# hip-satomi/microbeSEG

Measured on AMD Instinct MI355X. Metric: training crops/sec (256px), higher is better.
Workload: dtype f32; 1 GPU; BASELINE configs[1]: DU-Net distance-map training step, filters [64, 1024], 256x256 crops, per-GPU batch 32, fp32, relu/bn, SmoothL1x2 + Adam(amsgrad); global_batch=32, parallelism=dp1, launch=eager

## Files before the change

### include/mseg_hip.h

```cpp
#ifndef MSEG_HIP_H
#define MSEG_HIP_H

#include <stddef.h>
#include <stdint.h>

#ifdef __cplusplus
extern "C" {
#endif

#define MSEG_OK 0
#define MSEG_EINVAL (-1)
#define MSEG_ELAUNCH (-2)
#define MSEG_EWORKSPACE (-3)

#define MSEG_ACT_NONE 0
#define MSEG_ACT_RELU 1
#define MSEG_ACT_LEAKY 2
#define MSEG_ACT_ELU 3
#define MSEG_ACT_MISH 4

#define MSEG_NORM_BN 0
#define MSEG_NORM_GN 1
#define MSEG_NORM_IN 2

#define MSEG_ST_F32 0
#define MSEG_ST_BF16 1
typedef struct MsegSrc {
  const float* ptr;
  const float* scale;
  const float* shift;
  int32_t C;
  int32_t act;
  int32_t ss;
  int32_t dtype;
} MsegSrc;

#define MSEG_MODE_CONV 0
#define MSEG_MODE_TCONV 1
#define MSEG_EPI_PLAIN 0
#define MSEG_EPI_SCATTER2X2 1
#define MSEG_MORDER_LINEAR 0
#define MSEG_MORDER_PARITY 1
#define MSEG_PREC_F32 0
#define MSEG_PREC_BF16 1

typedef struct MsegIgemm {
  MsegSrc src[2];
  const float* w;
  const float* bias;
  float* dst0;
  float* dst1;
  int32_t nsrc, Cin, Kpad, Npad;
  int32_t NB, Hi, Wi, Ho, Wo;
  int32_t KH, KW, stride, pad, mode, morder;
  int32_t Ngemm, epi, split, ld0, ld1, acc0, acc1, Cq;
  int32_t precision;
  int32_t dst_dtype;
  void* ws;
  size_t ws_bytes;
  float* stats;
  int32_t stats_act;
  int32_t reserved0;
} MsegIgemm;

int mseg_igemm(const MsegIgemm* p, void* stream);

typedef struct MsegKernelInfo {
  char name[120];
  int32_t precision;
  int32_t launches;
  uint32_t grid, block;
  size_t workspace;
  int32_t stats_rows;
  int32_t reserved0;
} MsegKernelInfo;
int mseg_igemm_query(const MsegIgemm* p, MsegKernelInfo* info);
const char* mseg_last_kernel(void);
int mseg_f32_to_bf16(const float* src, uint16_t* dst, size_t n, void* stream);
size_t mseg_igemm_workspace_bytes(const MsegIgemm* p);
int mseg_igemm_set_persistent(int on);
int mseg_igemm_set_wide_tiles(int on);
int mseg_igemm_set_p8(int mode);

typedef struct MsegWgrad {
  MsegSrc P;
  MsegSrc Q[2];
  float* ws;
  float* dst;
  int32_t nq, Nch, Nch_store;
  int32_t NB, Hp, Wp, Hq, Wq;
  int32_t KH, KW, stride, pad;
  int32_t splits;
  int32_t phase;
  int32_t precision;
  int32_t reserved;
} MsegWgrad;

size_t mseg_wgrad_workspace_bytes(const MsegWgrad* p);
int mseg_wgrad(const MsegWgrad* p, void* stream);
int mseg_wgrad_query(const MsegWgrad* p, MsegKernelInfo* info);

int mseg_first_conv_fwd(const float* x4, const float* w, const float* bias, int N, int H, int W, int Cin, int Cout,
                        void* z, int z_dtype, void* stream);
#define MSEG_PIX_U8 0
#define MSEG_PIX_U16 1
#define MSEG_PIX_I32 2
#define MSEG_PIX_F32 3
int mseg_frame_minmax(const void* raw, int dtype, size_t npix, uint32_t* minmax, void* stream);
int mseg_first_conv_fwd_raw(const void* raw, int dtype, int H0, int W0, int pad_top, int pad_left, const uint32_t* minmax,
                            const float* w, const float* bias, int Cout, void* z, int z_dtype, void* stream);
int mseg_frame_normalize(const void* raw, int dtype, int H0, int W0, int pad_top, int pad_left, const uint32_t* minmax,
                         float* out, void* stream);
int mseg_frames_minmax(const void* raw, int dtype, int N, size_t npix_per_frame, uint32_t* minmax, void* stream);
int mseg_frames_normalize(const void* raw, int dtype, int N, int H0, int W0, int pad_top, int pad_left,
                          const uint32_t* minmax, float* out, void* stream);
size_t mseg_first_wgrad_workspace_bytes(int N, int H, int W, int Cout);
int mseg_first_wgrad(const float* x4, const void* dz, int dz_dtype, int N, int H, int W, int Cout, float* dW, void* ws,
                     void* stream);

int mseg_pack_weight(const float* src, float* dst, int T, int R, int Rpad, int C, int Cpad, int st, int sr, int sc,
                     void* stream);

typedef struct MsegPackJob {
  const float* src;
  float* dst;
  uint16_t* dst16;
  int32_t T, R, Rpad, C, Cpad, st, sr, sc;
  uint32_t first_block;
  uint32_t reserved;
} MsegPackJob;
unsigned mseg_pack_job_blocks(int T, int Rpad, int Cpad);
int mseg_pack_weights_multi(const MsegPackJob* jobs_dev, int njobs, unsigned total_blocks, void* stream);

size_t mseg_norm_workspace_bytes(int N, int HW, int C);
int mseg_norm_set_tails(int on);
int mseg_norm_set_finish(int on);
int mseg_norm_stats(const void* z, int N, int HW, int C, int st, int act, int norm, const float* gamma,
                    const float* beta, float eps, float* scale, float* shift, float* mean, float* rstd,
                    float* running_mean, float* running_var, float momentum, void* act_out, void* ws, void* stream);
int mseg_norm_stats_from_conv(const float* part, int rows, int C, long long count, const float* gamma, const float* beta,
                              float eps, float* scale, float* shift, float* mean, float* rstd, float* running_mean,
                              float* running_var, float momentum, void* ws, void* stream);
int mseg_activation(const void* z, int N, int HW, int C, int st, int act, void* act_out, void* stream);
int mseg_bn_eval_coeffs(const float* gamma, const float* beta, const float* running_mean,
                        const float* running_var, float eps, int C, float* scale, float* shift, void* stream);
int mseg_norm_bwd(const void* gy, const void* z, int N, int HW, int C, int st, int act, int norm, const float* gamma,
                  const float* mean, const float* rstd, void* dz, float* dgamma, float* dbeta, float* dbias,
                  const void* act_in , void* ws, void* stream);

int mseg_maxpool2x2_fwd(const MsegSrc* src, int N, int H, int W, float* out, void* stream);
int mseg_maxpool2x2_bwd(const MsegSrc* src, int N, int H, int W, const float* gout, float* gin, int accumulate,
                        void* stream);

int mseg_head_fwd(const MsegSrc* src, int N, int HW, const float* w, const float* b, int Co, float* out_nchw,
                  void* stream);
size_t mseg_head_bwd_workspace_bytes(int N, int HW, int C, int Co);
int mseg_head_bwd(const MsegSrc* src, int N, int HW, const float* w, int Co, const float* gout_nchw, void* gy,
                  int gy_dtype , float* dW, float* db, void* ws,
                  void* stream);

int mseg_softmax3_hwc(const float* logits_chw, int Hp, int Wp, int pad_y, int pad_x, float* probs_hwc, void* stream);

size_t mseg_loss_workspace_bytes(size_t n);
int mseg_regression_loss(const float* pred, const float* target, size_t n, int kind, float* loss_out,
                         void* ws, void* stream);
int mseg_regression_loss_bwd(const float* pred, const float* target, size_t n, int kind, const float* gscale_dev,
                             float* grad, void* stream);
int mseg_ce_dice_fwd(const float* logits, const int64_t* labels, int N, int HW, int with_dice, double* sums6,
                     double* ce_sum, void* ws, void* stream);
int mseg_ce_dice_bwd(const float* logits, const int64_t* labels, int N, int HW, int with_dice, const double* sums6,
                     double total_px, double dice_weight, const float* gscale_dev, float* grad, void* stream);

int mseg_polygons_find(const uint16_t* labels, int H, int W, int32_t* cand_px, int32_t* cand_id, int32_t* cand_len,
                       int capacity, int32_t* n_cand_dev, void* stream);
int mseg_polygons_trace(const uint16_t* labels, int H, int W, const int32_t* start_px, const int64_t* offsets, int n_poly,
                        int32_t* points_yx, void* stream);

int mseg_adam_amsgrad_step(float* p, const float* g, float* m, float* v, float* vmax, size_t n, double lr,
                           double beta1, double beta2, double eps, int step, void* stream);
int mseg_adam_amsgrad_step_dev(float* p, const float* g, float* m, float* v, float* vmax, size_t n, double* state,
                               double beta1, double beta2, double eps, void* stream);
int mseg_ranger_step(float* p, const float* g, float* m, float* v, float* slow, size_t n, int rows, double beta1,
                     double beta2, double eps, double step_lr, int rectified, int do_gc, int lookahead, double alpha,
                     void* stream);
typedef struct MsegRangerJob {
  float* p;
  const float* g;
  float* m;
  float* v;
  float* slow;
  uint64_t n;
  int32_t rows;
  float step_lr;
  uint32_t flags;
  uint32_t reserved;
} MsegRangerJob;
int mseg_ranger_step_multi(const MsegRangerJob* jobs, int njobs, double beta1, double beta2, double eps, double alpha,
                           void* stream);

size_t mseg_postproc_workspace_bytes(int H, int W);
int mseg_postproc_tuning(int heap_rows, int tile_small_px, int tile_large_px);
int mseg_postproc_set_const_stream(int on);
int mseg_distance_postprocess(const float* border, const float* cell, int H, int W, float th_cell, float th_seed,
                              int col_major_ids, uint16_t* labels, int32_t* n_instances_dev, int32_t* status_dev,
                              void* ws, size_t ws_bytes, void* stream);
int mseg_boundary_postprocess(const float* probs_hwc, int H, int W, uint16_t* labels, int32_t* n_instances_dev,
                              int32_t* status_dev, void* ws, size_t ws_bytes, void* stream);
int mseg_boundary_postprocess_pre(const float* probs_hwc, int H, int W, void* ws, size_t ws_bytes, void* stream);
int mseg_boundary_flood_batch(void* const* ws_list, int B, int H, int W, void* stream);
int mseg_boundary_postprocess_post(int H, int W, uint16_t* labels, int32_t* n_instances_dev, int32_t* status_dev, void* ws,
                                   size_t ws_bytes, void* stream);

int mseg_distance_postprocess_sweep(const float* border, const float* cell, int H, int W, const float* th_cell,
                                    const float* th_seed, int nth, int col_major_ids, uint16_t* labels,
                                    int32_t* n_instances_dev, int32_t* status_dev, void* ws, size_t ws_bytes,
                                    void* stream);

size_t mseg_postproc_batch_workspace_bytes(int N, int H, int W);
int mseg_distance_postprocess_batch(const float* border, const float* cell, int N, int H, int W, long long row_stride,
                                    long long frame_stride, float th_cell, float th_seed, int col_major_ids,
                                    uint16_t* labels, int32_t* n_instances_dev, int32_t* status_dev, void* ws,
                                    size_t ws_bytes, void* stream);

int mseg_aug_u16_to_f32(const uint16_t* in, float* out, size_t n, void* stream);
int mseg_aug_flip(const float* in, float* out, int N, int H, int W, const int32_t* codes_dev, void* stream);
int mseg_aug_affine(const float* in, float* out, int N, int H, int W, const float* mats_dev, const int32_t* apply_dev,
                    int nearest, void* stream);
int mseg_aug_blur(const float* in, float* tmp, float* out, int N, int H, int W, const float* sigmas_dev, void* stream);
int mseg_aug_stats(const float* in, int N, int H, int W, float* stats_dev, uint32_t* hist_dev, void* stream);
int mseg_aug_contrast_params(const float* stats_dev, const uint32_t* hist_dev, const float* choice_dev, int N, int HW,
                             float* par_dev, void* stream);
// ... 63 lines not shown
```

### microbeseg_amd/_lib.py

```python
import ctypes as C
import os
import pathlib

_HERE = pathlib.Path(__file__).resolve().parent
LIB_PATH = _HERE / "libmseg_hip.so"

ACT = {"none": 0, "relu": 1, "leakyrelu": 2, "elu": 3, "mish": 4}
NORM = {"bn": 0, "gn": 1, "in": 2}
MODE_CONV, MODE_TCONV = 0, 1
EPI_PLAIN, EPI_SCATTER2X2 = 0, 1
MORDER_LINEAR, MORDER_PARITY = 0, 1
ST_F32, ST_BF16 = 0, 1
PIX_U8, PIX_U16, PIX_I32, PIX_F32 = 0, 1, 2, 3


class MsegLibraryError(RuntimeError):
    pass


class MsegSrc(C.Structure):
    _fields_ = [("ptr", C.c_void_p), ("scale", C.c_void_p), ("shift", C.c_void_p),
                ("C", C.c_int32), ("act", C.c_int32), ("ss", C.c_int32), ("dtype", C.c_int32)]


class MsegIgemm(C.Structure):
    _fields_ = [("src", MsegSrc * 2), ("w", C.c_void_p), ("bias", C.c_void_p), ("dst0", C.c_void_p),
                ("dst1", C.c_void_p),
                ("nsrc", C.c_int32), ("Cin", C.c_int32), ("Kpad", C.c_int32), ("Npad", C.c_int32),
                ("NB", C.c_int32), ("Hi", C.c_int32), ("Wi", C.c_int32), ("Ho", C.c_int32), ("Wo", C.c_int32),
                ("KH", C.c_int32), ("KW", C.c_int32), ("stride", C.c_int32), ("pad", C.c_int32),
                ("mode", C.c_int32), ("morder", C.c_int32),
                ("Ngemm", C.c_int32), ("epi", C.c_int32), ("split", C.c_int32), ("ld0", C.c_int32),
                ("ld1", C.c_int32), ("acc0", C.c_int32), ("acc1", C.c_int32), ("Cq", C.c_int32),
                ("precision", C.c_int32), ("dst_dtype", C.c_int32), ("ws", C.c_void_p), ("ws_bytes", C.c_size_t),
                ("stats", C.c_void_p), ("stats_act", C.c_int32), ("reserved0", C.c_int32)]


class MsegWgrad(C.Structure):
    _fields_ = [("P", MsegSrc), ("Q", MsegSrc * 2), ("ws", C.c_void_p), ("dst", C.c_void_p),
                ("nq", C.c_int32), ("Nch", C.c_int32), ("Nch_store", C.c_int32),
                ("NB", C.c_int32), ("Hp", C.c_int32), ("Wp", C.c_int32), ("Hq", C.c_int32), ("Wq", C.c_int32),
                ("KH", C.c_int32), ("KW", C.c_int32), ("stride", C.c_int32), ("pad", C.c_int32),
                ("splits", C.c_int32), ("phase", C.c_int32), ("precision", C.c_int32), ("reserved", C.c_int32)]


class MsegKernelInfo(C.Structure):
    _fields_ = [("name", C.c_char * 120), ("precision", C.c_int32), ("launches", C.c_int32), ("grid", C.c_uint32),
                ("block", C.c_uint32), ("workspace", C.c_size_t), ("stats_rows", C.c_int32), ("reserved0", C.c_int32)]


class MsegPackJob(C.Structure):
    _fields_ = [("src", C.c_void_p), ("dst", C.c_void_p), ("dst16", C.c_void_p),
                ("T", C.c_int32), ("R", C.c_int32), ("Rpad", C.c_int32), ("C", C.c_int32), ("Cpad", C.c_int32),
                ("st", C.c_int32), ("sr", C.c_int32), ("sc", C.c_int32),
                ("first_block", C.c_uint32), ("reserved", C.c_uint32)]


class MsegRangerJob(C.Structure):
    _fields_ = [("p", C.c_void_p), ("g", C.c_void_p), ("m", C.c_void_p), ("v", C.c_void_p), ("slow", C.c_void_p),
                ("n", C.c_uint64), ("rows", C.c_int32), ("step_lr", C.c_float), ("flags", C.c_uint32),
                ("reserved", C.c_uint32)]


_P = C.c_void_p
_I = C.c_int
_F = C.c_float
_D = C.c_double
_SZ = C.c_size_t

SIGNATURES = {
    "mseg_igemm": (_I, [C.POINTER(MsegIgemm), _P]),
    "mseg_igemm_workspace_bytes": (_SZ, [C.POINTER(MsegIgemm)]),
    "mseg_igemm_query": (_I, [C.POINTER(MsegIgemm), C.POINTER(MsegKernelInfo)]),
    "mseg_last_kernel": (C.c_char_p, []),
    "mseg_igemm_set_persistent": (_I, [_I]),
    "mseg_igemm_set_wide_tiles": (_I, [_I]),
    "mseg_igemm_set_p8": (_I, [_I]),
    "mseg_f32_to_bf16": (_I, [_P, _P, _SZ, _P]),
    "mseg_first_conv_fwd": (_I, [_P, _P, _P, _I, _I, _I, _I, _I, _P, _I, _P]),
    "mseg_frame_minmax": (_I, [_P, _I, _SZ, _P, _P]),
    "mseg_first_conv_fwd_raw": (_I, [_P, _I, _I, _I, _I, _I, _P, _P, _P, _I, _P, _I, _P]),
    "mseg_frame_normalize": (_I, [_P, _I, _I, _I, _I, _I, _P, _P, _P]),
    "mseg_frames_minmax": (_I, [_P, _I, _I, _SZ, _P, _P]),
    "mseg_frames_normalize": (_I, [_P, _I, _I, _I, _I, _I, _I, _P, _P, _P]),
    "mseg_first_wgrad_workspace_bytes": (_SZ, [_I, _I, _I, _I]),
    "mseg_first_wgrad": (_I, [_P, _P, _I, _I, _I, _I, _I, _P, _P, _P]),
    "mseg_wgrad_workspace_bytes": (_SZ, [C.POINTER(MsegWgrad)]),
    "mseg_wgrad": (_I, [C.POINTER(MsegWgrad), _P]),
    "mseg_wgrad_query": (_I, [C.POINTER(MsegWgrad), C.POINTER(MsegKernelInfo)]),
    "mseg_pack_weight": (_I, [_P, _P, _I, _I, _I, _I, _I, _I, _I, _I, _P]),
    "mseg_pack_job_blocks": (C.c_uint, [_I, _I, _I]),
    "mseg_pack_weights_multi": (_I, [_P, _I, C.c_uint, _P]),
    "mseg_norm_workspace_bytes": (_SZ, [_I, _I, _I]),
    "mseg_norm_set_tails": (_I, [_I]),
    "mseg_norm_set_finish": (_I, [_I]),
    "mseg_norm_stats_from_conv": (_I, [_P, _I, _I, C.c_longlong, _P, _P, _F, _P, _P, _P, _P, _P, _P, _F, _P, _P]),
    "mseg_norm_stats": (_I, [_P, _I, _I, _I, _I, _I, _I, _P, _P, _F, _P, _P, _P, _P, _P, _P, _F, _P, _P, _P]),
    "mseg_activation": (_I, [_P, _I, _I, _I, _I, _I, _P, _P]),
    "mseg_bn_eval_coeffs": (_I, [_P, _P, _P, _P, _F, _I, _P, _P, _P]),
    "mseg_norm_bwd": (_I, [_P, _P, _I, _I, _I, _I, _I, _I, _P, _P, _P, _P, _P, _P, _P, _P, _P, _P]),
    "mseg_maxpool2x2_fwd": (_I, [C.POINTER(MsegSrc), _I, _I, _I, _P, _P]),
    "mseg_maxpool2x2_bwd": (_I, [C.POINTER(MsegSrc), _I, _I, _I, _P, _P, _I, _P]),
    "mseg_head_fwd": (_I, [C.POINTER(MsegSrc), _I, _I, _P, _P, _I, _P, _P]),
    "mseg_head_bwd_workspace_bytes": (_SZ, [_I, _I, _I, _I]),
    "mseg_head_bwd": (_I, [C.POINTER(MsegSrc), _I, _I, _P, _I, _P, _P, _I, _P, _P, _P, _P]),
    "mseg_softmax3_hwc": (_I, [_P, _I, _I, _I, _I, _P, _P]),
    "mseg_loss_workspace_bytes": (_SZ, [_SZ]),
    "mseg_regression_loss": (_I, [_P, _P, _SZ, _I, _P, _P, _P]),
    "mseg_regression_loss_bwd": (_I, [_P, _P, _SZ, _I, _P, _P, _P]),
    "mseg_ce_dice_fwd": (_I, [_P, _P, _I, _I, _I, _P, _P, _P, _P]),
    "mseg_ce_dice_bwd": (_I, [_P, _P, _I, _I, _I, _P, C.c_double, C.c_double, _P, _P, _P]),
    "mseg_adam_amsgrad_step": (_I, [_P, _P, _P, _P, _P, _SZ, _D, _D, _D, _D, _I, _P]),
    "mseg_adam_amsgrad_step_dev": (_I, [_P, _P, _P, _P, _P, _SZ, _P, _D, _D, _D, _P]),
    "mseg_ranger_step": (_I, [_P, _P, _P, _P, _P, _SZ, _I, _D, _D, _D, _D, _I, _I, _I, _D, _P]),
    "mseg_ranger_step_multi": (_I, [_P, _I, _D, _D, _D, _D, _P]),
    "mseg_postproc_workspace_bytes": (_SZ, [_I, _I]),
    "mseg_postproc_tuning": (_I, [_I, _I, _I]),
    "mseg_postproc_set_const_stream": (_I, [_I]),
    "mseg_distance_postprocess": (_I, [_P, _P, _I, _I, _F, _F, _I, _P, _P, _P, _P, _SZ, _P]),
    "mseg_boundary_postprocess": (_I, [_P, _I, _I, _P, _P, _P, _P, _SZ, _P]),
    "mseg_boundary_postprocess_pre": (_I, [_P, _I, _I, _P, _SZ, _P]),
    "mseg_boundary_flood_batch": (_I, [C.POINTER(C.c_void_p), _I, _I, _I, _P]),
    "mseg_boundary_postprocess_post": (_I, [_I, _I, _P, _P, _P, _P, _SZ, _P]),
    "mseg_distance_postprocess_sweep": (_I, [_P, _P, _I, _I, C.POINTER(C.c_float), C.POINTER(C.c_float), _I, _I, _P, _P,
                                             _P, _P, _SZ, _P]),
    "mseg_postproc_batch_workspace_bytes": (_SZ, [_I, _I, _I]),
    "mseg_distance_postprocess_batch": (_I, [_P, _P, _I, _I, _I, C.c_longlong, C.c_longlong, _F, _F, _I, _P, _P, _P, _P,
                                             _SZ, _P]),
    "mseg_aug_u16_to_f32": (_I, [_P, _P, _SZ, _P]),
    "mseg_aug_flip": (_I, [_P, _P, _I, _I, _I, _P, _P]),
    "mseg_aug_affine": (_I, [_P, _P, _I, _I, _I, _P, _P, _I, _P]),
    "mseg_aug_blur": (_I, [_P, _P, _P, _I, _I, _I, _P, _P]),
    "mseg_aug_stats": (_I, [_P, _I, _I, _I, _P, _P, _P]),
    "mseg_aug_contrast_params": (_I, [_P, _P, _P, _I, _I, _P, _P]),
    "mseg_aug_contrast": (_I, [_P, _P, _I, _I, _I, _P, _P]),
    "mseg_aug_clahe_workspace_bytes": (_SZ, [_I]),
    "mseg_aug_clahe": (_I, [_P, _P, _I, _I, _I, _P, _P, _P]),
    "mseg_aug_noise_normalize": (_I, [_P, _P, _I, _I, _I, _P, _P, C.c_uint32, _F, _F, _P]),
    "mseg_clahe_workspace_bytes": (_SZ, [_I, _I, _I]),
    "mseg_clahe_u16": (_I, [_P, _I, _I, _I, _I, _P, _P, _I, _P, _SZ, _P]),
    "mseg_label_boundary": (_I, [_P, _I, _I, _I, _I, _P, _P]),
    "mseg_label_distance_workspace_bytes": (_SZ, [_I, _I, _I]),
    "mseg_label_distance": (_I, [_P, _I, _I, _I, _I, _P, _P, _P, _SZ, _P]),
    "mseg_label_bottom_hat": (_I, [_P, _I, _I, _I, _P, _P, _P, _SZ, _P]),
    "mseg_label_cell_distance": (_I, [_P, _I, _I, _I, _I, _F, _P, _P, _SZ, _P]),
    "mseg_label_j4": (_I, [_P, _I, _I, _I, _I, _I, _P, _P, _P]),
    "mseg_label_major_axis_workspace_bytes": (_SZ, [_I]),
    "mseg_label_max_major_axis": (_I, [_P, _I, _I, _I, _P, _P, _SZ, _P]),
    "mseg_eval_workspace_bytes": (_SZ, [_I, _I]),
    "mseg_eval_relabel": (_I, [_P, _I, _I, _I, _P, _P, _P, _SZ, _P]),
    "mseg_eval_pair_counts": (_I, [_P, _P, _I, _I, _I, _I, _P, _P, _P, _P]),
    "mseg_polygons_find": (_I, [_P, _I, _I, _P, _P, _P, _I, _P, _P]),
    "mseg_polygons_trace": (_I, [_P, _I, _I, _P, _P, _I, _P, _P]),
    "mseg_roi_fill_workspace_bytes": (_SZ, [_I]),
    "mseg_roi_fill": (_I, [_P, _P, _P, _I, _I, _I, _I, _P, _P, _SZ, _P]),
    "mseg_roi_outline": (_I, [_P, _P, _P, _I, C.c_int64, _I, _I, _I, _P, _P]),
    "mseg_stack_relabel_workspace_bytes": (_SZ, [_I, _I, _I]),
    "mseg_stack_relabel": (_I, [_P, _I, _I, _I, _I, _P, _P, _P, _SZ, _P]),
    "mseg_region_stats_workspace_bytes": (_SZ, [C.c_int64]),
    "mseg_region_stats": (_I, [_P, _I, _I, _I, _P, C.c_int64, _P, _P, _P, _P, _P, _SZ, _P]),
    "mseg_overlay_workspace_bytes": (_SZ, []),
    "mseg_overlay_rgb": (_I, [_P, _I, _I, _I, _I, _I, _P, _P, _P, _SZ, _P]),
    "mseg_frame_stats": (_I, [_P, _I, _SZ, _P, _P]),
    "mseg_crops_extract": (_I, [_P, _I, _I, _I, _I, _P, _I, _I, _I, _I, _P, _P, _P, _P, _P]),
    "mseg_crop_census_workspace_bytes": (_SZ, []),
    "mseg_crop_census": (_I, [_P, _I, _I, _I, _I, _I, _I, _I, _I, _P, _P, _P, _SZ, _P]),
    "mseg_crops_overlay": (_I, [_P, _P, _P, _I, _I, _P]),
    "mseg_version": (_I, []),
    "mseg_strerror": (C.c_char_p, [_I]),
    "mseg_last_hip_error": (_I, []),
}

_lib = None


def load():
    global _lib
    if _lib is not None:
        return _lib
    import torch
    path = os.environ.get("MSEG_HIP_LIB", str(LIB_PATH))
    if not os.path.exists(path):
        raise MsegLibraryError(
# ... 24 lines not shown
```

### microbeseg_amd/csrc/api_misc.hip

```cpp
#include "common.h"
#include <string.h>

static thread_local int g_last_hip_error = 0;

extern "C" void mseg_set_hip_error(int e) { g_last_hip_error = e; }
extern "C" int mseg_last_hip_error(void) { return g_last_hip_error; }
extern "C" int mseg_version(void) { return 100; }
extern "C" const char* mseg_strerror(int code) {
  switch (code) {
    case MSEG_OK: return "ok";
    case MSEG_EINVAL: return "invalid argument or unsupported shape";
    case MSEG_ELAUNCH: return "HIP launch/runtime error (see mseg_last_hip_error)";
    case MSEG_EWORKSPACE: return "workspace too small";
    default: return "unknown error";
  }
}

static thread_local int g_dry = 0;
static thread_local MsegKernelInfo g_call;
static thread_local char g_last_kernel[sizeof(g_call.name)] = "";

extern "C" int mseg_dispatch_dry(void) { return g_dry; }
extern "C" void mseg_dispatch_begin(int dry) {
  g_dry = dry;
  memset(&g_call, 0, sizeof(g_call));
}
extern "C" void mseg_dispatch_end(MsegKernelInfo* info) {
  if (!g_dry && g_call.name[0]) memcpy(g_last_kernel, g_call.name, sizeof(g_last_kernel));
  if (info) *info = g_call;
  g_dry = 0;
}
extern "C" void mseg_dispatch_note(int precision, size_t workspace) {
  g_call.precision = precision;
  g_call.workspace = workspace;
}
extern "C" void mseg_dispatch_note_stats(int rows) { g_call.stats_rows = rows; }
extern "C" void mseg_note_launch(const char* kernel, unsigned grid, unsigned block, int aux) {
  g_call.launches += 1;
  if (aux || g_call.name[0]) return;
  size_t n = strlen(kernel);
  if (n >= 2 && kernel[0] == '(' && kernel[n - 1] == ')') { ++kernel; n -= 2; }
  if (n >= sizeof(g_call.name)) n = sizeof(g_call.name) - 1;
  memcpy(g_call.name, kernel, n);
  g_call.name[n] = 0;
  g_call.grid = grid;
  g_call.block = block;
}
extern "C" const char* mseg_last_kernel(void) { return g_last_kernel; }
```

### microbeseg_amd/csrc/common.h

```cpp
#pragma once
#include <hip/hip_runtime.h>
#include <stdint.h>
#include "../../include/mseg_hip.h"

extern "C" void mseg_set_hip_error(int e);
extern "C" int mseg_dispatch_dry(void);

#define MSEG_LAUNCH_CHECK()                           \
  do {                                                \
    if (mseg_dispatch_dry()) break;                   \
    hipError_t e__ = hipGetLastError();               \
    if (e__ != hipSuccess) {                          \
      mseg_set_hip_error((int)e__);                   \
      return MSEG_ELAUNCH;                            \
    }                                                 \
  } while (0)

extern "C" void mseg_note_launch(const char* kernel, unsigned grid, unsigned block, int aux);
extern "C" void mseg_dispatch_begin(int dry);
extern "C" void mseg_dispatch_end(MsegKernelInfo* info);
extern "C" void mseg_dispatch_note(int precision, size_t workspace);
extern "C" void mseg_dispatch_note_stats(int rows);
#define MSEG_KL(K, grid_, block_, shmem_, st_, ...)                                              \
  do {                                                                                           \
    mseg_note_launch(#K, (unsigned)(grid_).x, (unsigned)(block_).x, 0);                          \
    if (!mseg_dispatch_dry()) hipLaunchKernelGGL(K, grid_, block_, shmem_, st_, ##__VA_ARGS__);    \
  } while (0)
#define MSEG_KL_AUX(K, grid_, block_, shmem_, st_, ...)                                          \
  do {                                                                                           \
    mseg_note_launch(#K, (unsigned)(grid_).x, (unsigned)(block_).x, 1);                          \
    if (!mseg_dispatch_dry()) hipLaunchKernelGGL(K, grid_, block_, shmem_, st_, ##__VA_ARGS__);    \
  } while (0)

typedef float f32x16 __attribute__((ext_vector_type(16)));
typedef float f32x4 __attribute__((ext_vector_type(4)));

__device__ __forceinline__ float mseg_softplus(float x) {
  return x > 20.f ? x : log1pf(expf(x));
}

template <bool FAST>
__device__ __forceinline__ float mish_fwd(float x) {
  if (x > 20.f) return x;
  const float w = FAST ? __expf(x) : expf(x);
  const float n = w * (w + 2.f);
  return FAST ? x * n * __frcp_rn(n + 2.f) : x * (n / (n + 2.f));
}
template <bool FAST>
__device__ __forceinline__ float mish_bwd(float x) {
  if (x > 20.f) return 1.f;
  const float w = FAST ? __expf(x) : expf(x);
  const float n = w * (w + 2.f);
  const float r = FAST ? __frcp_rn(n + 2.f) : 1.f / (n + 2.f);
  return n * r + 4.f * x * w * (w + 1.f) * r * r;
}

template <int ACT>
__device__ __forceinline__ float act_fwd_t(float x) {
  if (ACT == MSEG_ACT_RELU) return x > 0.f ? x : 0.f;
  if (ACT == MSEG_ACT_LEAKY) return x > 0.f ? x : 0.01f * x;
  if (ACT == MSEG_ACT_ELU) return x > 0.f ? x : expm1f(x);
  if (ACT == MSEG_ACT_MISH) return mish_fwd<false>(x);
  return x;
}

__device__ __forceinline__ float act_fwd(float x, int act) {
  switch (act) {
    case MSEG_ACT_RELU: return act_fwd_t<MSEG_ACT_RELU>(x);
    case MSEG_ACT_LEAKY: return act_fwd_t<MSEG_ACT_LEAKY>(x);
    case MSEG_ACT_ELU: return act_fwd_t<MSEG_ACT_ELU>(x);
    case MSEG_ACT_MISH: return act_fwd_t<MSEG_ACT_MISH>(x);
    default: return x;
  }
}

__device__ __forceinline__ float act_bwd(float z, int act) {
  switch (act) {
    case MSEG_ACT_RELU: return z > 0.f ? 1.f : 0.f;
    case MSEG_ACT_LEAKY: return z > 0.f ? 1.f : 0.01f;
    case MSEG_ACT_ELU: return z > 0.f ? 1.f : expf(z);
    case MSEG_ACT_MISH: return mish_bwd<false>(z);
    default: return 1.f;
  }
}

__device__ __forceinline__ float act_fwd_fast(float x, int act) {
  if (act == MSEG_ACT_MISH) return mish_fwd<true>(x);
  if (act == MSEG_ACT_ELU) return x > 0.f ? x : __expf(x) - 1.f;
  return act_fwd(x, act);
}
__device__ __forceinline__ float act_bwd_fast(float z, int act) {
  if (act == MSEG_ACT_MISH) return mish_bwd<true>(z);
  if (act == MSEG_ACT_ELU) return z > 0.f ? 1.f : __expf(z);
  return act_bwd(z, act);
}

template <bool FAST>
__device__ __forceinline__ void act_pair(float z, int act, float& a, float& d) {
  if (act == MSEG_ACT_MISH) {
    if (z > 20.f) { a = z; d = 1.f; return; }
    const float w = FAST ? __expf(z) : expf(z);
    const float n = w * (w + 2.f);
    if (FAST) {
      const float r = __frcp_rn(n + 2.f);
      a = z * n * r;
      d = n * r + 4.f * z * w * (w + 1.f) * r * r;
    } else {
      const float r = 1.f / (n + 2.f);
      a = z * (n / (n + 2.f));
      d = n * r + 4.f * z * w * (w + 1.f) * r * r;
    }
    return;
  }
  a = FAST ? act_fwd_fast(z, act) : act_fwd(z, act);
  d = FAST ? act_bwd_fast(z, act) : act_bwd(z, act);
}

__device__ __forceinline__ float4 act_fwd4(float4 v, int act) {
  if (act == MSEG_ACT_NONE) return v;
  if (act == MSEG_ACT_RELU) {
    v.x = fmaxf(v.x, 0.f); v.y = fmaxf(v.y, 0.f); v.z = fmaxf(v.z, 0.f); v.w = fmaxf(v.w, 0.f);
    return v;
  }
  v.x = act_fwd(v.x, act); v.y = act_fwd(v.y, act); v.z = act_fwd(v.z, act); v.w = act_fwd(v.w, act);
  return v;
}

__device__ __forceinline__ float4 src_load4(const MsegSrc& s, size_t e);

__device__ __forceinline__ float4 src_transform4(float4 v, const MsegSrc& s, int n, int c) {
  v = act_fwd4(v, s.act);
  if (s.scale) {
    const float4 sc = *reinterpret_cast<const float4*>(s.scale + (size_t)n * s.ss + c);
    const float4 sh = *reinterpret_cast<const float4*>(s.shift + (size_t)n * s.ss + c);
    v.x = v.x * sc.x + sh.x; v.y = v.y * sc.y + sh.y; v.z = v.z * sc.z + sh.z; v.w = v.w * sc.w + sh.w;
  }
  return v;
}

typedef __bf16 mseg_bf16x2 __attribute__((ext_vector_type(2)));

__device__ __forceinline__ float bf16_lo(unsigned v) { return __uint_as_float(v << 16); }
__device__ __forceinline__ float bf16_hi(unsigned v) { return __uint_as_float(v & 0xffff0000u); }
__device__ __forceinline__ unsigned pack_bf16x2(float a, float b) {
  mseg_bf16x2 v;
  v[0] = (__bf16)a; v[1] = (__bf16)b;
  return __builtin_bit_cast(unsigned, v);
}
__device__ __forceinline__ float4 bf16x4_to_f32(uint2 v) {
  return make_float4(bf16_lo(v.x), bf16_hi(v.x), bf16_lo(v.y), bf16_hi(v.y));
}
__device__ __forceinline__ uint2 f32x4_to_bf16(float4 v) { return make_uint2(pack_bf16x2(v.x, v.y), pack_bf16x2(v.z, v.w)); }

template <bool S16>
__device__ __forceinline__ float4 ld_f4(const void* base, size_t e) {
  if (S16) return bf16x4_to_f32(*reinterpret_cast<const uint2*>(reinterpret_cast<const uint16_t*>(base) + e));
  return *reinterpret_cast<const float4*>(reinterpret_cast<const float*>(base) + e);
}
template <bool S16>
__device__ __forceinline__ void st_f4(void* base, size_t e, float4 v) {
  if (S16) *reinterpret_cast<uint2*>(reinterpret_cast<uint16_t*>(base) + e) = f32x4_to_bf16(v);
  else *reinterpret_cast<float4*>(reinterpret_cast<float*>(base) + e) = v;
}
__device__ __forceinline__ float4 ld_f4_rt(const void* base, size_t e, int bf16) {
  return bf16 ? ld_f4<true>(base, e) : ld_f4<false>(base, e);
}
// ... 31 lines not shown
```

### microbeseg_amd/csrc/igemm.hip

```cpp
#include "common.h"
#include "igemm_common.h"
#include "bf16_affine.h"

int igemm_p8_try(const MsegIgemm& p, int tr, int m_fastest, int cus, hipStream_t st);

__device__ float g_ident_scale[MSEG_MAX_CH];
__device__ float g_ident_shift[MSEG_MAX_CH];
__global__ void init_ident_kernel() {
  for (int i = blockIdx.x * blockDim.x + threadIdx.x; i < MSEG_MAX_CH; i += gridDim.x * blockDim.x) {
    g_ident_scale[i] = 1.f;
    g_ident_shift[i] = 0.f;
  }
}


template <int BM, int BN, bool PER_SAMPLE, bool GENERIC_ACT>
__global__ __launch_bounds__(256) void igemm_kernel(const MsegIgemm p) {
  using Cfg = IgemmCfg<BM, BN>;
  constexpr int STAGE = (BM + BN) * LDS_STRIDE;
  __shared__ __attribute__((aligned(16))) float lds[2 * STAGE + 4];
  unsigned* tapmask_s = reinterpret_cast<unsigned*>(lds + 2 * STAGE);

  const int tid = threadIdx.x;
  const int lane = tid & 63;
// ... 357 lines not shown
      const int cls = m0 / (M >> 2);
      py = cls >> 1; px = cls & 1;
    }
    for (int tt = 0; tt < T; ++tt) {
      const int ky_ = tt / p.KW, kx_ = tt - ky_ * p.KW;
      const bool live = (((py - geom.dir * (ky_ - geom.pad)) | (px - geom.dir * (kx_ - geom.pad))) & geom.sh) == 0;
      if (live) {
        const unsigned long long e = (unsigned long long)(tt | (ky_ << 4) | (kx_ << 6));
        if (nlive < 8) taplist |= e << (8 * nlive); else taplist_hi |= e << (8 * (nlive - 8));
        ++nlive;
      }
    }
  }
  auto tap_at = [&](int j) -> unsigned { return (unsigned)((j < 8 ? taplist >> (8 * j) : taplist_hi >> (8 * (j - 8))) & 0xffull); };
  int chunk = 0, j = 0;
  const int nsteps = nchunks * nlive;
  unsigned e0 = tap_at(0);
  issue(0, (int)(e0 & 15u), (int)((e0 >> 4) & 3u), (int)(e0 >> 6));
  commit(lds, lds + BM * LDS_STRIDE);
  __syncthreads();
  int cur = 0;
  const int li = lane & 31, lh = lane >> 5;
  for (int step = 0; step < nsteps; ++step) {
    if (step + 1 < nsteps) {
      j += 1;
      if (j >= nlive) { j = 0; ++chunk; }
    }
    e0 = tap_at(j);
    issue(chunk, (int)(e0 & 15u), (int)((e0 >> 4) & 3u), (int)(e0 >> 6));

    const float* As = lds + cur * STAGE;
    const float* Bs = As + BM * LDS_STRIDE;
#pragma unroll
    for (int kk = 0; kk < KC / 8; ++kk) {
      float4 af[Cfg::MB], bf[Cfg::NB];
#pragma unroll
      for (int a = 0; a < Cfg::MB; ++a)
        af[a] = *reinterpret_cast<const float4*>(As + (wm * Cfg::TM + a * 32 + li) * LDS_STRIDE + kk * 8 + lh * 4);
#pragma unroll
      for (int b = 0; b < Cfg::NB; ++b)
        bf[b] = *reinterpret_cast<const float4*>(Bs + (wn * Cfg::TN + b * 32 + li) * LDS_STRIDE + kk * 8 + lh * 4);
#pragma unroll
      for (int a = 0; a < Cfg::MB; ++a)
#pragma unroll
        for (int b = 0; b < Cfg::NB; ++b) {
          acc[a][b] = __builtin_amdgcn_mfma_f32_32x32x2f32(af[a].x, bf[b].x, acc[a][b], 0, 0, 0);
          acc[a][b] = __builtin_amdgcn_mfma_f32_32x32x2f32(af[a].y, bf[b].y, acc[a][b], 0, 0, 0);
          acc[a][b] = __builtin_amdgcn_mfma_f32_32x32x2f32(af[a].z, bf[b].z, acc[a][b], 0, 0, 0);
          acc[a][b] = __builtin_amdgcn_mfma_f32_32x32x2f32(af[a].w, bf[b].w, acc[a][b], 0, 0, 0);
        }
    }
    if (SB) {
      __syncthreads();
      commit(lds, lds + BM * LDS_STRIDE);
      __syncthreads();
    } else {
      float* An = lds + (cur ^ 1) * STAGE;
      commit(An, An + BM * LDS_STRIDE);
      __syncthreads();
      cur ^= 1;
    }
  }
  igemm_epilogue<IgemmCfg<BM, BN>>(acc, m0, n0, wm, wn, lane, M);
}

template <int BN>
struct HaloCfg {
  static constexpr int WN = (BN >= 128) ? 4 : 2;
  static constexpr int WM = 8 / WN;
  static constexpr int TM = 128 / WM, TN = BN / WN;
  static constexpr int MB = TM / 32, NB = TN / 32;
  static constexpr int BROWS = BN / 64;
};

template <int BN, int TR>
__global__ __launch_bounds__(512, 2) void igemm_halo_kernel(const MsegIgemm p, int tw_log2, int ksplit,
                                                            int chunks_per_split) {
  constexpr int BM = 128;
  using Cfg = HaloCfg<BN>;
  constexpr int HMAX = 264;
  constexpr int HL = (HMAX * 8 + 511) / 512;
  constexpr int ASTAGE = HMAX * LDS_STRIDE;
  constexpr int BSTAGE = BN * LDS_STRIDE;
  __shared__ __attribute__((aligned(16))) float lds[ASTAGE + 2 * BSTAGE];
  float* const Abuf = lds;
  float* const Bbuf = lds + ASTAGE;

  const int tid = threadIdx.x, lane = tid & 63, wave = tid >> 6;
  const int wm = wave / Cfg::WN, wn = wave % Cfg::WN;
  const int li = lane & 31, lh = lane >> 5;
  const int srow = tid >> 3, scol = tid & 7;
  const int TW = 1 << tw_log2, TH = BM >> tw_log2, HW2 = TW + 2;
  const int HROWS = (TH + 2) * HW2;
  const int H = p.Hi, W = p.Wi;
  const int M = p.NB * H * W;
  const int tiles_x = W >> tw_log2, tiles_y = (H + TH - 1) / TH;
  const int ntiles_n = (p.Ngemm + BN - 1) / BN;
  const int lid_all = (int)xcd_logical_id(blockIdx.x, gridDim.x);
  const int ntiles_all = (int)gridDim.x / ksplit;
  const int kz = lid_all / ntiles_all;
  const int lid = lid_all - kz * ntiles_all;
  const int tile_m = lid / ntiles_n, tile_n = lid - tile_m * ntiles_n;
  const int img = tile_m / (tiles_x * tiles_y);
  const int trem = tile_m - img * (tiles_x * tiles_y);
  const int ty = trem / tiles_x, tx = trem - ty * tiles_x;
  const int oy0 = ty * TH, ox0 = tx * TW, n0 = tile_n * BN;
  const int band0 = oy0 > 0 ? oy0 - 1 : 0;
  const int band_rows = (oy0 + TH + 1 < H ? oy0 + TH + 1 : H) - band0;
  const bool conv = p.mode == MSEG_MODE_CONV;

  int hpix[HL];
  unsigned hvalid = 0u;
#pragma unroll
  for (int j = 0; j < HL; ++j) {
    const int hrow = srow + 64 * j;
    const int hy = hrow / HW2, hx = hrow - hy * HW2;
    const int iy = oy0 - 1 + hy, ix = ox0 - 1 + hx;
    const bool ok = (hrow < HROWS) & (iy >= 0) & (iy < H) & (ix >= 0) & (ix < W);
    hpix[j] = (iy - band0) * W + ix;
    hvalid |= (unsigned)ok << j;
  }
  int abase[Cfg::MB];
#pragma unroll
  for (int a = 0; a < Cfg::MB; ++a) {
    const int i = wm * Cfg::TM + a * 32 + li;
    abase[a] = ((i >> tw_log2) * HW2 + (i & (TW - 1))) * LDS_STRIDE + lh * 4;
  }

  f32x16 acc[Cfg::MB][Cfg::NB];
#pragma unroll
  for (int a = 0; a < Cfg::MB; ++a)
#pragma unroll
    for (int b = 0; b < Cfg::NB; ++b)
#pragma unroll
      for (int r = 0; r < 16; ++r) acc[a][b][r] = 0.f;

  const int nchunks = (p.Cin + KC - 1) / KC;
  const int C0 = p.src[0].C;
  const unsigned OOB = 0x80000000u;
  const int C1 = p.nsrc > 1 ? p.src[1].C : p.src[0].C;
  const float* const base0 = p.src[0].ptr + ((size_t)img * H + band0) * W * p.src[0].C;
  const float* const base1 = (p.nsrc > 1 ? p.src[1].ptr : p.src[0].ptr) + ((size_t)img * H + band0) * W * C1;
  const __amdgpu_buffer_rsrc_t rs0 = __builtin_amdgcn_make_buffer_rsrc(const_cast<float*>(base0), 0,
                                                                        band_rows * W * p.src[0].C * 4, 0x00020000);
  const __amdgpu_buffer_rsrc_t rs1 = __builtin_amdgcn_make_buffer_rsrc(const_cast<float*>(base1), 0,
                                                                        band_rows * W * C1 * 4, 0x00020000);
  const __amdgpu_buffer_rsrc_t rsw = __builtin_amdgcn_make_buffer_rsrc(const_cast<float*>(p.w), 0,
                                                                        9 * p.Npad * p.Kpad * 4, 0x00020000);
  unsigned wvoff[Cfg::BROWS];
#pragma unroll
  for (int i = 0; i < Cfg::BROWS; ++i) wvoff[i] = ((unsigned)(n0 + srow + 64 * i) * (unsigned)p.Kpad + scol * 4u) * 4u;

  float4 rh[HL], rb[Cfg::BROWS], rsc, rsh;
  unsigned hlive = 0u;
  int ract = 0;
  bool cur_s1 = false;

  auto issue_halo = [&](int chunk) {
    const int c = chunk * KC + scol * 4;
    cur_s1 = (p.nsrc > 1) && (chunk * KC >= C0);
    const MsegSrc& s = cur_s1 ? p.src[1] : p.src[0];
    const unsigned sC4 = (unsigned)s.C * 4u;
    const unsigned soff = (unsigned)(chunk * KC - (cur_s1 ? C0 : 0)) * 4u + scol * 16u;
    hlive = (c < p.Cin) ? hvalid : 0u;
#pragma unroll
    for (int j = 0; j < HL; ++j) {
      const bool ok = (hlive >> j) & 1u;
      const unsigned vo = ok ? (unsigned)hpix[j] * sC4 + soff : OOB;
      const f32x4 v = cur_s1 ? __builtin_bit_cast(f32x4, __builtin_amdgcn_raw_buffer_load_b128(rs1, vo, 0, 0))
                             : __builtin_bit_cast(f32x4, __builtin_amdgcn_raw_buffer_load_b128(rs0, vo, 0, 0));
      rh[j] = make_float4(v[0], v[1], v[2], v[3]);
    }
    if (TR != 0) {
      ract = s.act;
      const bool has_aff = s.scale != nullptr;
      const float* scp = has_aff ? s.scale : g_ident_scale;
      const float* shp = has_aff ? s.shift : g_ident_shift;
      const unsigned cl = (c < p.Cin) ? (unsigned)(cur_s1 ? c - C0 : c) : 0u;
      const size_t o = (size_t)img * (has_aff ? (unsigned)s.ss : 0u) + cl;
      rsc = *reinterpret_cast<const float4*>(scp + o);
      rsh = *reinterpret_cast<const float4*>(shp + o);
    }
  };

  auto commit_halo = [&](float* As) {
    const float lo = (ract == MSEG_ACT_RELU) ? 0.f : -3.402823466e38f;
#pragma unroll
    for (int j = 0; j < HL; ++j) {
      const int hrow = srow + 64 * j;
      if (hrow < HMAX) {
        float4 v = rh[j];
        if (TR != 0) {
          if (TR == 2) v = act_fwd4(v, ract);
          else { v.x = clamp_lo(v.x, lo); v.y = clamp_lo(v.y, lo); v.z = clamp_lo(v.z, lo); v.w = clamp_lo(v.w, lo); }
          const float m = ((hlive >> j) & 1u) ? 1.f : 0.f;
          v.x = (v.x * rsc.x + rsh.x) * m; v.y = (v.y * rsc.y + rsh.y) * m;
          v.z = (v.z * rsc.z + rsh.z) * m; v.w = (v.w * rsc.w + rsh.w) * m;
        }
        *reinterpret_cast<float4*>(As + hrow * LDS_STRIDE + scol * 4) = v;
      }
    }
  };

  auto issue_b = [&](int chunk, int t) {
    const unsigned wso = ((unsigned)t * (unsigned)p.Npad * (unsigned)p.Kpad + (unsigned)chunk * KC) * 4u;
#pragma unroll
    for (int i = 0; i < Cfg::BROWS; ++i) {
      const f32x4 v = __builtin_bit_cast(f32x4, __builtin_amdgcn_raw_buffer_load_b128(rsw, wvoff[i], wso, 0));
      rb[i] = make_float4(v[0], v[1], v[2], v[3]);
    }
  };
  auto commit_b = [&](float* Bs) {
#pragma unroll
    for (int i = 0; i < Cfg::BROWS; ++i)
      *reinterpret_cast<float4*>(Bs + (srow + 64 * i) * LDS_STRIDE + scol * 4) = rb[i];
  };

  const int c_begin = kz * chunks_per_split;
  const int c_end = (c_begin + chunks_per_split < nchunks) ? c_begin + chunks_per_split : nchunks;
  issue_halo(c_begin);
  issue_b(c_begin, 0);
  commit_halo(Abuf);
  commit_b(Bbuf);
  __syncthreads();

  int bsel = 0;
  for (int chunk = c_begin; chunk < c_end; ++chunk) {
    const float* As = Abuf;
    const bool more_chunks = chunk + 1 < c_end;
    for (int t = 0; t < 9; ++t) {
      if (t == 0 && more_chunks) issue_halo(chunk + 1);
      const bool last = (t == 8) && !more_chunks;
      issue_b(t == 8 ? (more_chunks ? chunk + 1 : chunk) : chunk, last ? 8 : (t == 8 ? 0 : t + 1));

      const int ky = t / 3, kx = t - 3 * ky;
      const int toff = ((conv ? ky : 2 - ky) * HW2 + (conv ? kx : 2 - kx)) * LDS_STRIDE;
      const float* Bs = Bbuf + bsel * BSTAGE;
#pragma unroll
      for (int kk = 0; kk < KC / 8; ++kk) {
        float4 af[Cfg::MB], bf[Cfg::NB];
#pragma unroll
        for (int a = 0; a < Cfg::MB; ++a)
          af[a] = *reinterpret_cast<const float4*>(As + abase[a] + toff + kk * 8);
#pragma unroll
        for (int b = 0; b < Cfg::NB; ++b)
          bf[b] = *reinterpret_cast<const float4*>(Bs + (wn * Cfg::TN + b * 32 + li) * LDS_STRIDE + kk * 8 + lh * 4);
#pragma unroll
        for (int a = 0; a < Cfg::MB; ++a)
#pragma unroll
          for (int b = 0; b < Cfg::NB; ++b) {
            acc[a][b] = __builtin_amdgcn_mfma_f32_32x32x2f32(af[a].x, bf[b].x, acc[a][b], 0, 0, 0);
            acc[a][b] = __builtin_amdgcn_mfma_f32_32x32x2f32(af[a].y, bf[b].y, acc[a][b], 0, 0, 0);
            acc[a][b] = __builtin_amdgcn_mfma_f32_32x32x2f32(af[a].z, bf[b].z, acc[a][b], 0, 0, 0);
            acc[a][b] = __builtin_amdgcn_mfma_f32_32x32x2f32(af[a].w, bf[b].w, acc[a][b], 0, 0, 0);
          }
      }
      commit_b(Bbuf + (bsel ^ 1) * BSTAGE);
      if (t == 8 && more_chunks) {
        __syncthreads();
        commit_halo(Abuf);
      }
      __syncthreads();
      bsel ^= 1;
    }
  }
  igemm_epilogue<Cfg>(acc, 0, n0, wm, wn, lane, M * ksplit, tw_log2, img + kz * p.NB, oy0, ox0);
}

typedef __bf16 bf16x8 __attribute__((ext_vector_type(8)));
typedef __bf16 bf16x4 __attribute__((ext_vector_type(4)));
#define HB_STRIDE 40

template <int BN, int BM>
struct HaloCfgM {
  static constexpr int WN = (BN >= 128) ? 4 : 2;
  static constexpr int WM = 8 / WN;
  static constexpr int TM = BM / WM, TN = BN / WN;
  static constexpr int MB = TM / 32, NB = TN / 32;
  static constexpr int BROWS = BN / 64;
};

template <int BN, int TR, bool S16, int BM>
__device__ __forceinline__ void igemm_halo_bf16_body(const MsegIgemm& p, int tw_log2, int ksplit, int chunks_per_split,
                                                     int m_fastest) {
  using Cfg = HaloCfgM<BN, BM>;
  constexpr int HMAX = BM == 128 ? 204 : 612;
  constexpr int SQ = S16 ? 4 : 8;
  constexpr int SROWS = 512 / SQ;
  constexpr int HL = (HMAX + SROWS - 1) / SROWS;
  constexpr int ASTAGE = HMAX * HB_STRIDE;
  constexpr int BSTAGE = 3 * BN * HB_STRIDE;
  __shared__ __attribute__((aligned(16))) __bf16 lds[ASTAGE + 2 * BSTAGE];
  __bf16* const Abuf = lds;
  __bf16* const Bbuf = lds + ASTAGE;

  const int tid = threadIdx.x, lane = tid & 63, wave = tid >> 6;
  const int wm = wave / Cfg::WN, wn = wave % Cfg::WN;
  const int li = lane & 31, lh = lane >> 5;
  const int srow = tid / SQ, scol = tid % SQ;
  const int brow = tid >> 2, bcol = tid & 3;
  const int TW = 1 << tw_log2, TH = BM >> tw_log2, HW2 = TW + 2;
  const int HROWS = (TH + 2) * HW2;
  const int H = p.Hi, W = p.Wi;
  const int M = p.NB * H * W;
  const int tiles_x = W >> tw_log2, tiles_y = (H + TH - 1) / TH;
  const int ntiles_n = (p.Ngemm + BN - 1) / BN;
  const int lid_all = (int)xcd_logical_id(blockIdx.x, gridDim.x);
  const int ntiles_all = (int)gridDim.x / ksplit;
  const int kz = lid_all / ntiles_all;
  const int lid = lid_all - kz * ntiles_all;
  const int ntiles_m = ntiles_all / ntiles_n;
  const int tile_m = m_fastest ? lid % ntiles_m : lid / ntiles_n;
  const int tile_n = m_fastest ? lid / ntiles_m : lid - tile_m * ntiles_n;
// ... 1750 lines not shown
  if (ks <= 1 || (p.Ngemm & 3)) return 0;
  return (size_t)ks * p.NB * p.Hi * p.Wi * p.Ngemm * sizeof(float);
}

static int igemm_dispatch(const MsegIgemm* pp, void* stream) {
  if (!pp) return MSEG_EINVAL;
  const MsegIgemm& p = *pp;
  if (p.nsrc < 1 || p.nsrc > 2) return MSEG_EINVAL;
  int csum = 0;
  for (int i = 0; i < p.nsrc; ++i) {
    if (check_src(p.src[i])) return MSEG_EINVAL;
    csum += p.src[i].C;
  }
  if (csum != p.Cin) return MSEG_EINVAL;
  if (!p.w || !p.dst0 || p.Kpad < p.Cin || (p.Kpad % KC) || p.Npad < p.Ngemm || (p.Npad % 128)) return MSEG_EINVAL;
  if (p.Cin > MSEG_MAX_CH) return MSEG_EINVAL;
  if (p.NB <= 0 || p.Hi <= 0 || p.Wi <= 0 || p.Ho <= 0 || p.Wo <= 0) return MSEG_EINVAL;
  if (p.KH <= 0 || p.KW <= 0 || p.KH * p.KW > 16) return MSEG_EINVAL;
  if (p.stride != 1 && p.stride != 2) return MSEG_EINVAL;
  if (p.mode != MSEG_MODE_CONV && p.mode != MSEG_MODE_TCONV) return MSEG_EINVAL;
  if (p.morder == MSEG_MORDER_PARITY && ((p.Ho | p.Wo) & 1)) return MSEG_EINVAL;
  if (p.Ngemm <= 0) return MSEG_EINVAL;
  if (p.precision != MSEG_PREC_F32 && p.precision != MSEG_PREC_BF16) return MSEG_EINVAL;
  if (p.dst_dtype != MSEG_ST_F32 && p.dst_dtype != MSEG_ST_BF16) return MSEG_EINVAL;
  const bool s16 = p.src[0].dtype == MSEG_ST_BF16;
  if (p.nsrc > 1 && p.src[1].dtype != p.src[0].dtype) return MSEG_EINVAL;
  if ((s16 || p.dst_dtype == MSEG_ST_BF16) && p.precision != MSEG_PREC_BF16) return MSEG_EINVAL;
  if (p.dst_dtype == MSEG_ST_BF16) {
    if ((p.Ngemm | p.ld0 | p.ld1 | p.Cq) & 1) return MSEG_EINVAL;
    if (p.split < p.Ngemm && (p.split & 1)) return MSEG_EINVAL;
    if (((uintptr_t)p.dst0 | (uintptr_t)p.dst1) & 3) return MSEG_EINVAL;
  }
  if (p.epi == MSEG_EPI_SCATTER2X2) {
    if (p.Cq <= 0 || p.Ngemm != 4 * p.Cq || p.morder != MSEG_MORDER_LINEAR) return MSEG_EINVAL;
  } else if (p.epi == MSEG_EPI_PLAIN) {
    if (p.split < p.Ngemm && !p.dst1) return MSEG_EINVAL;
  } else {
    return MSEG_EINVAL;
  }
  const long long M = (long long)p.NB * p.Ho * p.Wo;
  if (M <= 0 || M > 0x7fffffffLL) return MSEG_EINVAL;
  hipStream_t st = (hipStream_t)stream;
  mseg_dispatch_note(p.precision, 0);
  static bool ident_ready[64] = {false};
  int devid = 0;
  const bool dry = mseg_dispatch_dry() != 0;
  if (!dry) {
    if (hipGetDevice(&devid) != hipSuccess || devid < 0 || devid >= 64) return MSEG_ELAUNCH;
    if (!ident_ready[devid]) {
      MSEG_KL_AUX(init_ident_kernel, dim3(8), dim3(256), 0, st);
      MSEG_LAUNCH_CHECK();
      ident_ready[devid] = true;
    }
  }
  bool per_sample = false, generic = false;
  for (int i = 0; i < p.nsrc; ++i) {
    if (p.src[i].scale && p.src[i].ss != 0) per_sample = true;
    if (p.src[i].act != MSEG_ACT_NONE && p.src[i].act != MSEG_ACT_RELU) generic = true;
  }
  const bool wide = p.Ngemm > 64;
  const int BMv = 128, BNv = wide ? 128 : 64;
  const long long tiles = ((M + BMv - 1) / BMv) * ((p.Ngemm + BNv - 1) / BNv);
  if (tiles > 0x7fffffffLL) return MSEG_EINVAL;
  const dim3 grid((unsigned)tiles), block(256);
  bool fast = (p.mode == MSEG_MODE_CONV) || (p.stride == 1) ||
              (p.morder == MSEG_MORDER_PARITY && (M % (4 * BMv)) == 0);
  bool plain = true, band_fits = true;
  for (int i = 0; i < p.nsrc; ++i) {
    if (((128LL / p.Wo + 3) * p.stride + p.KH) * p.Wi * p.src[i].C * 4 >= 0x7ffffff0LL) fast = false;
    if (34LL * p.Wi * p.src[i].C * 4 >= 0x80000000LL) band_fits = false;
    if (p.src[i].act != MSEG_ACT_NONE || p.src[i].scale) plain = false;
  }
  bool common = true;
  if ((long long)p.KH * p.KW * p.Npad * p.Kpad * 4 >= 0x80000000LL) common = false;
  if (p.KH > 4 || p.KW > 4) common = false;
  if (p.nsrc > 1 && (p.src[0].C % KC)) common = false;
  fast = fast && common;
  int tw_log2 = 6;
  long long htiles = 0;
  if (common && band_fits && halo_geometry(p, BNv, &tw_log2, &htiles) && htiles <= 0x7fffffffLL) {
    const int tr = plain ? 0 : (generic ? 2 : 1);
    int cps = 0;
    int ks = halo_ksplit(htiles, (p.Cin + KC - 1) / KC, &cps);
    const size_t need = (size_t)ks * (size_t)M * (size_t)p.Ngemm * sizeof(float);
    if (ks > 1 && (!p.ws || p.ws_bytes < need || (p.Ngemm & 3) || (p.split & 3) || htiles * ks > 0x7fffffffLL)) {
      ks = 1;
      cps = (p.Cin + KC - 1) / KC;
    }
    MsegIgemm q = p;
    if (ks > 1) {
      q.dst0 = (float*)p.ws; q.dst1 = nullptr; q.ld0 = p.Ngemm; q.ld1 = 0; q.split = p.Ngemm; q.acc0 = 0; q.acc1 = 0;
      q.bias = nullptr;
      q.dst_dtype = MSEG_ST_F32;
    }
    mseg_dispatch_note(p.precision, ks > 1 ? need : 0);
    const dim3 hgrid((unsigned)(htiles * ks));
#define MSEG_HALO(BN_, TR_) MSEG_KL((igemm_halo_kernel<BN_, TR_>), hgrid, dim3(512), 0, st, q, tw_log2, ks, cps)
    const int m_fastest = ((long long)9 * p.Kpad * p.Ngemm * 2 > (2ll << 20)) && (p.Ngemm > BNv) ? 1 : 0;
#define MSEG_HALO16(BN_, TR_)                                                                                          \
  do {                                                                                                                 \
    if (s16) MSEG_KL((igemm_halo_bf16_kernel<BN_, TR_, true>), hgrid, dim3(512), 0, st, q, tw_log2, ks, cps, m_fastest); \
    else MSEG_KL((igemm_halo_bf16_kernel<BN_, TR_, false>), hgrid, dim3(512), 0, st, q, tw_log2, ks, cps, m_fastest);    \
  } while (0)
#define MSEG_HALO16W4(TR_)                                                                                             \
  do {                                                                                                                 \
    if (s16) MSEG_KL((igemm_halo_bf16w4_kernel<TR_, true>), hgrid, dim3(256), 0, st, q, tw_log2, ks, cps, m_fastest);    \
    else MSEG_KL((igemm_halo_bf16w4_kernel<TR_, false>), hgrid, dim3(256), 0, st, q, tw_log2, ks, cps, m_fastest);       \
  } while (0)
    int p8rc = 0;
    if (p.precision == MSEG_PREC_BF16 && s16 && !wide && g_c64p_on && p.nsrc == 1 && p.Cin == 64 && p.Kpad == 64 &&
        ks == 1 && tw_log2 <= 5 && p.split >= p.Ngemm && htiles >= 4 * (long long)c64p_workgroups()) {
      const int wgs = c64p_workgroups();
      const dim3 pgrid((unsigned)wgs);
#define MSEG_C64P(TR_)                                                                                                        \
  do {                                                                                                                         \
    if (q.dst_dtype == MSEG_ST_BF16) MSEG_KL((igemm_c64p_bf16_kernel<TR_, true>), pgrid, dim3(512), 0, st, q, tw_log2, (int)htiles); \
    else MSEG_KL((igemm_c64p_bf16_kernel<TR_, false>), pgrid, dim3(512), 0, st, q, tw_log2, (int)htiles);               \
  } while (0)
      if (tr == 0) MSEG_C64P(0); else if (tr == 1) MSEG_C64P(1); else MSEG_C64P(2);
#undef MSEG_C64P
    } else if (p.precision == MSEG_PREC_BF16 && !wide && g_c64p_on && p.Cin >= 128 && ks == 1 && tw_log2 >= 4 &&
               halo512_tiles(p, tw_log2) >= 2 * (long long)c64p_workgroups()) {
      const dim3 mgrid((unsigned)halo512_tiles(p, tw_log2));
#define MSEG_HALO512(TR_)                                                                                                      \
  do {                                                                                                                         \
    if (s16) MSEG_KL((igemm_halo_bf16m512_kernel<TR_, true>), mgrid, dim3(512), 0, st, q, tw_log2, 1, cps, 0);      \
    else MSEG_KL((igemm_halo_bf16m512_kernel<TR_, false>), mgrid, dim3(512), 0, st, q, tw_log2, 1, cps, 0);         \
  } while (0)
      if (tr == 0) MSEG_HALO512(0); else if (tr == 1) MSEG_HALO512(1); else MSEG_HALO512(2);
#undef MSEG_HALO512
    } else if (p.precision == MSEG_PREC_BF16 && wide && s16 && ks == 1 &&
               (p8rc = igemm_p8_try(q, tr, m_fastest, c64p_workgroups(), st)) != 0) {
      if (p8rc < 0) return p8rc;
    } else if (p.precision == MSEG_PREC_BF16 && wide && s16 && g_w4m_on && ks == 1 && tw_log2 >= 3 &&
               halo_big_tiles(p, tw_log2, 256) * ((p.Ngemm + 127) / 128) >= 2 * (long long)c64p_workgroups()) {
      const dim3 mgrid((unsigned)(halo_big_tiles(p, tw_log2, 256) * ((p.Ngemm + 127) / 128)));
#define MSEG_HALOW4M(TR_) \
  MSEG_KL((igemm_halo_bf16w4m_kernel<TR_, true>), mgrid, dim3(256), 0, st, q, tw_log2, 1, cps, m_fastest)
      if (tr == 0) MSEG_HALOW4M(0); else if (tr == 1) MSEG_HALOW4M(1); else MSEG_HALOW4M(2);
#undef MSEG_HALOW4M
    } else if (p.precision == MSEG_PREC_BF16) {
      if (wide) { if (tr == 0) MSEG_HALO16W4(0); else if (tr == 1) MSEG_HALO16W4(1); else MSEG_HALO16W4(2); }
      else      { if (tr == 0) MSEG_HALO16(64, 0); else if (tr == 1) MSEG_HALO16(64, 1); else MSEG_HALO16(64, 2); }
    } else if (wide) { if (tr == 0) MSEG_HALO(128, 0); else if (tr == 1) MSEG_HALO(128, 1); else MSEG_HALO(128, 2); }
    else      { if (tr == 0) MSEG_HALO(64, 0); else if (tr == 1) MSEG_HALO(64, 1); else MSEG_HALO(64, 2); }
#undef MSEG_HALO
#undef MSEG_HALO16
#undef MSEG_HALO16W4
    MSEG_LAUNCH_CHECK();
    if (ks > 1) {
      const size_t total = (size_t)M * (size_t)(p.Ngemm >> 2);
      size_t blocks = (total + 255) / 256;
      if (blocks > 16384) blocks = 16384;
      MSEG_KL_AUX(igemm_splitk_reduce_kernel, dim3((unsigned)blocks), dim3(256), 0, st, (const float*)p.ws, ks,
                         (size_t)M, p.Ngemm, p.bias, p.dst0, p.ld0, p.acc0, p.dst1, p.ld1, p.acc1,
                         p.split < p.Ngemm ? p.split : p.Ngemm, p.dst_dtype == MSEG_ST_BF16 ? 1 : 0);
      MSEG_LAUNCH_CHECK();
    }
    return MSEG_OK;
  }
  if (p.precision == MSEG_PREC_BF16 && s16 && g_c64p_on && p.epi == MSEG_EPI_SCATTER2X2 && p.KH == 1 && p.KW == 1 &&
      p.stride == 1 && p.pad == 0 && p.mode == MSEG_MODE_CONV && p.nsrc == 1 && p.Cin == 128 && p.Kpad == 128 &&
      p.Cq == 64 && p.Ngemm == 256 && !p.acc0 && (p.Wi % 32) == 0 && (((long long)p.Hi * p.Wi) % 128) == 0 &&
      M / 128 >= 4 * (long long)c64p_workgroups()) {
    const int tr = plain ? 0 : (generic ? 2 : 1);
    const dim3 pgrid((unsigned)c64p_workgroups());
    const int nt = (int)(M / 128);
#define MSEG_CTP(TR_)                                                                                                \
  do {                                                                                                               \
    if (p.dst_dtype == MSEG_ST_BF16) MSEG_KL((igemm_ctp_bf16_kernel<TR_, true>), pgrid, dim3(512), 0, st, p, nt); \
    else MSEG_KL((igemm_ctp_bf16_kernel<TR_, false>), pgrid, dim3(512), 0, st, p, nt);                     \
  } while (0)
    if (tr == 0) MSEG_CTP(0); else if (tr == 1) MSEG_CTP(1); else MSEG_CTP(2);
#undef MSEG_CTP
    MSEG_LAUNCH_CHECK();
    return MSEG_OK;
  }
  if (p.precision == MSEG_PREC_BF16 && s16 && g_c64p_on && p.epi == MSEG_EPI_SCATTER2X2 && p.KH == 1 && p.KW == 1 &&
      p.stride == 1 && p.pad == 0 && p.mode == MSEG_MODE_CONV && p.nsrc == 1 && p.Cin == 256 && p.Kpad == 256 &&
      p.Cq == 128 && p.Ngemm == 512 && !p.acc0 && p.Wi >= 32 && (((long long)p.Hi * p.Wi) % 64) == 0 &&
      (c64p_workgroups() & 3) == 0 && M / 64 >= 4 * (long long)(c64p_workgroups() / 4)) {
    const int tr = plain ? 0 : (generic ? 2 : 1);
    const dim3 pgrid((unsigned)c64p_workgroups());
    const int nt = (int)(M / 64);
#define MSEG_CTP2(TR_)                                                                                               \
  do {                                                                                                               \
    if (p.dst_dtype == MSEG_ST_BF16) MSEG_KL((igemm_ctp2_bf16_kernel<TR_, true>), pgrid, dim3(512), 0, st, p, nt); \
    else MSEG_KL((igemm_ctp2_bf16_kernel<TR_, false>), pgrid, dim3(512), 0, st, p, nt);                    \
  } while (0)
    if (tr == 0) MSEG_CTP2(0); else if (tr == 1) MSEG_CTP2(1); else MSEG_CTP2(2);
#undef MSEG_CTP2
    MSEG_LAUNCH_CHECK();
    return MSEG_OK;
  }
  if (p.precision == MSEG_PREC_BF16 && s16 && g_c64p_on && plain && p.epi == MSEG_EPI_PLAIN && p.KH == 2 && p.KW == 2 &&
      p.stride == 2 && p.pad == 0 && p.mode == MSEG_MODE_CONV && p.morder == MSEG_MORDER_LINEAR && p.nsrc == 1 &&
      p.Cin == 64 && p.Kpad == 64 && p.Ngemm == 128 && p.split >= p.Ngemm && !p.acc0 && !p.bias && (p.Wo % 32) == 0 &&
      p.Hi == 2 * p.Ho && p.Wi == 2 * p.Wo && (M % 64) == 0 && M / 64 >= 4 * (long long)c64p_workgroups()) {
    const dim3 pgrid((unsigned)c64p_workgroups());
    if (p.dst_dtype == MSEG_ST_BF16) MSEG_KL((igemm_ctd_bf16_kernel<true>), pgrid, dim3(512), 0, st, p, (int)(M / 64));
    else MSEG_KL((igemm_ctd_bf16_kernel<false>), pgrid, dim3(512), 0, st, p, (int)(M / 64));
    MSEG_LAUNCH_CHECK();
    return MSEG_OK;
  }
  if (p.precision == MSEG_PREC_BF16) {
    if (!fast) return MSEG_EINVAL;
    const int tr = plain ? 0 : (generic ? 2 : 1);
#define MSEG_FAST16_LAUNCH(BM_, BN_, TR_, PS_)                                                          \
  do {                                                                                                  \
    if (s16) MSEG_KL((igemm_fast_bf16_kernel<BM_, BN_, TR_, PS_, true>), grid, block, 0, st, p);   \
    else MSEG_KL((igemm_fast_bf16_kernel<BM_, BN_, TR_, PS_, false>), grid, block, 0, st, p);      \
  } while (0)
#define MSEG_FAST16_TILE(BM_, BN_)                                                        \
  do {                                                                                    \
    if (tr == 0) MSEG_FAST16_LAUNCH(BM_, BN_, 0, false);                                  \
    else if (tr == 1) { if (per_sample) MSEG_FAST16_LAUNCH(BM_, BN_, 1, true); else MSEG_FAST16_LAUNCH(BM_, BN_, 1, false); } \
    else { if (per_sample) MSEG_FAST16_LAUNCH(BM_, BN_, 2, true); else MSEG_FAST16_LAUNCH(BM_, BN_, 2, false); }              \
  } while (0)
    if (wide) MSEG_FAST16_TILE(128, 128); else MSEG_FAST16_TILE(128, 64);
#undef MSEG_FAST16_TILE
#undef MSEG_FAST16_LAUNCH
    MSEG_LAUNCH_CHECK();
    return MSEG_OK;
  }
  if (fast) {
    const int tr = plain ? 0 : (generic ? 2 : 1);
    const int live_taps = (p.mode == MSEG_MODE_TCONV && p.stride == 2) ? ((p.KH + 1) / 2) * ((p.KW + 1) / 2) : p.KH * p.KW;
    const bool short_k = ((p.Cin + KC - 1) / KC) * live_taps <= 8;
#define MSEG_FAST_LAUNCH(BM_, BN_, TR_, PS_)                                                              \
  do {                                                                                                    \
    if (short_k) MSEG_KL((igemm_fast_kernel<BM_, BN_, TR_, PS_, true>), grid, block, 0, st, p); \
    else MSEG_KL((igemm_fast_kernel<BM_, BN_, TR_, PS_, false>), grid, block, 0, st, p);        \
  } while (0)
#define MSEG_FAST_TILE(BM_, BN_)                                                          \
  do {                                                                                    \
    if (tr == 0) MSEG_FAST_LAUNCH(BM_, BN_, 0, false);                                    \
    else if (tr == 1) { if (per_sample) MSEG_FAST_LAUNCH(BM_, BN_, 1, true); else MSEG_FAST_LAUNCH(BM_, BN_, 1, false); } \
    else { if (per_sample) MSEG_FAST_LAUNCH(BM_, BN_, 2, true); else MSEG_FAST_LAUNCH(BM_, BN_, 2, false); }              \
  } while (0)
    if (wide) MSEG_FAST_TILE(128, 128); else MSEG_FAST_TILE(128, 64);
#undef MSEG_FAST_TILE
#undef MSEG_FAST_LAUNCH
    MSEG_LAUNCH_CHECK();
// ... 122 lines not shown
```

### microbeseg_amd/csrc/norm.hip

```cpp
#include "common.h"
#include <stdlib.h>

struct NormGeom {
  int N, HW, C, chunks, rows_per_chunk;
  int cw, slices;
};

#define NORM_CTR_BYTES 65536
#define NORM_CTR_MAX (NORM_CTR_BYTES / 4)

static NormGeom norm_geom(int N, int HW, int C, int vec = 4) {
  NormGeom g;
  g.N = N; g.HW = HW; g.C = C;
  const int C4 = C / vec;
  g.cw = C4 < 16 ? (C4 > 0 ? C4 : 1) : 16;
  g.slices = (C4 + g.cw - 1) / g.cw;
  const int rpi = 256 / g.cw;
  const int min_rows = 8 * rpi;
  const int target = 1024;
  int want = (target + N * g.slices - 1) / (N * g.slices > 0 ? N * g.slices : 1);
  int chunks = HW / min_rows;
  if (chunks > want) chunks = want;
  if (chunks < 1) chunks = 1;
  g.rows_per_chunk = (HW + chunks - 1) / chunks;
  g.chunks = (HW + g.rows_per_chunk - 1) / g.rows_per_chunk;
  return g;
}

static inline int norm_vec(int st) { return st == MSEG_ST_BF16 ? 8 : 4; }

extern "C" size_t mseg_norm_workspace_bytes(int N, int HW, int C) {
  if (N <= 0 || HW <= 0 || C <= 0) return 0;
  NormGeom g4 = norm_geom(N, HW, C, 4), g8 = norm_geom(N, HW, C, 8);
  const int chunks = g4.chunks > g8.chunks ? g4.chunks : g8.chunks;
  return NORM_CTR_BYTES + ((size_t)N * chunks * 3 * C + (size_t)3 * N * C + (size_t)2 * N * C + (size_t)32 * C) * sizeof(double);
}

template <bool S16>
struct NormVec {
  static constexpr int V = S16 ? 8 : 4;
  uint4 raw;
  __device__ __forceinline__ void load(const void* base, size_t e) {
    if (S16) raw = *reinterpret_cast<const uint4*>(reinterpret_cast<const uint16_t*>(base) + e);
    else raw = *reinterpret_cast<const uint4*>(reinterpret_cast<const float*>(base) + e);
  }
  __device__ __forceinline__ void get(float (&v)[V]) const {
    if (S16) {
      v[0] = bf16_lo(raw.x); v[1] = bf16_hi(raw.x); v[2] = bf16_lo(raw.y); v[3] = bf16_hi(raw.y);
      v[V - 4] = bf16_lo(raw.z); v[V - 3] = bf16_hi(raw.z); v[V - 2] = bf16_lo(raw.w); v[V - 1] = bf16_hi(raw.w);
    } else {
      v[0] = __uint_as_float(raw.x); v[1] = __uint_as_float(raw.y); v[2] = __uint_as_float(raw.z); v[3] = __uint_as_float(raw.w);
    }
  }
  static __device__ __forceinline__ void round(float (&v)[V]) {
    if (S16) {
#pragma unroll
      for (int j = 0; j < V; j += 2) {
        const uint32_t r = pack_bf16x2(v[j], v[j + 1]);
        v[j] = bf16_lo(r); v[j + 1] = bf16_hi(r);
      }
    }
  }
  static __device__ __forceinline__ void put(void* base, size_t e, float (&v)[V]) {
    if (S16) {
      uint4 r;
      r.x = pack_bf16x2(v[0], v[1]); r.y = pack_bf16x2(v[2], v[3]);
      r.z = pack_bf16x2(v[V - 4], v[V - 3]); r.w = pack_bf16x2(v[V - 2], v[V - 1]);
      *reinterpret_cast<uint4*>(reinterpret_cast<uint16_t*>(base) + e) = r;
      v[0] = bf16_lo(r.x); v[1] = bf16_hi(r.x); v[2] = bf16_lo(r.y); v[3] = bf16_hi(r.y);
      v[V - 4] = bf16_lo(r.z); v[V - 3] = bf16_hi(r.z); v[V - 2] = bf16_lo(r.w); v[V - 1] = bf16_hi(r.w);
    } else {
      *reinterpret_cast<float4*>(reinterpret_cast<float*>(base) + e) = make_float4(v[0], v[1], v[2], v[3]);
    }
  }
};

typedef __attribute__((address_space(1))) unsigned long long norm_gu64;
typedef __attribute__((address_space(1))) unsigned norm_gu32;
__device__ __forceinline__ void norm_st_sc1(double* p, double v) {
  __hip_atomic_store((norm_gu64*)p, (unsigned long long)__double_as_longlong(v), __ATOMIC_RELAXED, __HIP_MEMORY_SCOPE_AGENT);
}
__device__ __forceinline__ double norm_ld_sc1(const double* p) {
  return __longlong_as_double((long long)__hip_atomic_load((norm_gu64*)const_cast<double*>(p), __ATOMIC_RELAXED,
                                                           __HIP_MEMORY_SCOPE_AGENT));
}
__device__ __forceinline__ bool norm_arrive(unsigned* ctr, unsigned expected, int tid, int* s_flag) {
  asm volatile("s_waitcnt vmcnt(0)" ::: "memory");
  __syncthreads();
  if (tid == 0) {
    const unsigned ticket = __hip_atomic_fetch_add((norm_gu32*)ctr, 1u, __ATOMIC_RELAXED, __HIP_MEMORY_SCOPE_AGENT);
    const int last = ticket == expected - 1u;
    if (last) {
      __hip_atomic_store((norm_gu32*)ctr, 0u, __ATOMIC_RELAXED, __HIP_MEMORY_SCOPE_AGENT);
      __builtin_amdgcn_fence(__ATOMIC_ACQUIRE, "agent");
    }
    *s_flag = last;
    asm volatile("s_waitcnt vmcnt(0)" ::: "memory");
  }
  __syncthreads();
  return *s_flag != 0;
}

#define NORM_TAIL_NONE 0
#define NORM_TAIL_BN_FWD 1
#define NORM_TAIL_PS_FWD 2
#define NORM_TAIL_BN_BWD 3
#define NORM_TAIL_COLSUM 4
struct NormTail {
  int kind, norm;
  unsigned* ctr;
  double* nc;
  const float* gamma; const float* beta;
  float eps, momentum;
  float *scale, *shift, *mean_out, *rstd_out, *running_mean, *running_var;
  const float *mean, *rstd;
  float *k1, *k2, *k3, *dgamma, *dbeta, *colsum;
};

template <int MODE, bool S16, bool AIO>
__global__ __launch_bounds__(256) void norm_pass_kernel(const void* __restrict__ z, const void* __restrict__ gy,
                                                        void* __restrict__ dz, const float* __restrict__ k1,
                                                        const float* __restrict__ k2, const float* __restrict__ k3,
                                                        int kss, NormGeom g, int act, double* __restrict__ part,
                                                        void* __restrict__ aio, const NormTail t) {
  constexpr int V = S16 ? 8 : 4;
  __shared__ double red[256 * 2 * V];
  __shared__ int s_flag;
  const int tid = threadIdx.x;
  const int chunk = blockIdx.x, n = blockIdx.y, slice = blockIdx.z;
  const int C4 = g.C / V;
  const int CW = g.cw;
  const int rpi = 256 / CW;
  const int cq = tid % CW, r0 = tid / CW;
  const int row_begin = chunk * g.rows_per_chunk;
  int row_end = row_begin + g.rows_per_chunk;
  if (row_end > g.HW) row_end = g.HW;
  constexpr int NS = (MODE == 2) ? 1 : 2;
  double* pout = part + ((size_t)n * g.chunks + chunk) * 3 * g.C;
  const int c4 = slice * CW + cq;
  const bool active = (c4 < C4) && (r0 < rpi);
  double s0[V], s1[V];
#pragma unroll
  for (int j = 0; j < V; ++j) { s0[j] = 0.0; s1[j] = 0.0; }
  if (active) {
    const int c = c4 * V;
    float a1[V], a2[V], a3[V];
    if (MODE == 2) {
#pragma unroll
      for (int j = 0; j < V; ++j) {
        a1[j] = k1[(size_t)n * kss + c + j]; a2[j] = k2[(size_t)n * kss + c + j]; a3[j] = k3[(size_t)n * kss + c + j];
      }
    }
    constexpr int U = (MODE == 0 && !AIO) ? 8 : !S16 ? 4 : MODE == 1 ? (AIO ? 2 : 4) : MODE == 2 ? 2 : 4;
    for (int r = row_begin + r0; r < row_end; r += rpi * U) {
      NormVec<S16> zv[U], gv[U], av[U];
      bool ok[U];
      float p0[V], p1[V];
#pragma unroll
      for (int j = 0; j < V; ++j) { p0[j] = 0.f; p1[j] = 0.f; }
#pragma unroll
      for (int u = 0; u < U; ++u) {
        const int ru = r + u * rpi;
        ok[u] = ru < row_end;
        const size_t off = ((size_t)n * g.HW + (ok[u] ? ru : r)) * g.C + c;
        if (MODE != 1 || !AIO) zv[u].load(z, off);
        if (MODE == 1 && AIO) av[u].load(aio, off);
        if (MODE == 1 || MODE == 2) gv[u].load(gy, off);
      }
#pragma unroll
      for (int u = 0; u < U; ++u) {
        if (!ok[u]) continue;
        const size_t off = ((size_t)n * g.HW + r + u * rpi) * g.C + c;
        float zf[V], a4[V];
        if (MODE != 1 || !AIO) zv[u].get(zf);
        if (MODE == 2 && AIO) {
          float gf[V], d[V];
          gv[u].get(gf);
#pragma unroll
          for (int j = 0; j < V; ++j) act_pair<S16>(zf[j], act, a4[j], d[j]);
          NormVec<S16>::round(a4);
#pragma unroll
          for (int j = 0; j < V; ++j) d[j] = (a1[j] * gf[j] + a2[j] * a4[j] + a3[j]) * d[j];
          NormVec<S16>::put(dz, off, d);
#pragma unroll
          for (int j = 0; j < V; ++j) p0[j] += d[j];
          continue;
        }
        if (MODE == 1 && AIO) av[u].get(a4);
        else {
          if (S16 && act != MSEG_ACT_NONE && act != MSEG_ACT_RELU) {
#pragma unroll
            for (int j = 0; j < V; ++j) a4[j] = act_fwd_fast(zf[j], act);
          } else {
#pragma unroll
            for (int j = 0; j < V; j += 4) {
              const float4 t4 = act_fwd4(make_float4(zf[j], zf[j + 1], zf[j + 2], zf[j + 3]), act);
              a4[j] = t4.x; a4[j + 1] = t4.y; a4[j + 2] = t4.z; a4[j + 3] = t4.w;
            }
          }
        }
        if ((MODE == 0 || MODE == 3) && AIO)
          NormVec<S16>::put(aio, off, a4);
        if (MODE == 3) continue;
        if (MODE == 0) {
#pragma unroll
          for (int j = 0; j < V; ++j) { p0[j] += a4[j]; p1[j] = fmaf(a4[j], a4[j], p1[j]); }
        } else {
          float gf[V];
          gv[u].get(gf);
          if (MODE == 1) {
#pragma unroll
            for (int j = 0; j < V; ++j) { p0[j] += gf[j]; p1[j] = fmaf(gf[j], a4[j], p1[j]); }
          } else {
            float d[V];
#pragma unroll
            for (int j = 0; j < V; ++j)
              d[j] = (a1[j] * gf[j] + a2[j] * a4[j] + a3[j]) * (S16 ? act_bwd_fast(zf[j], act) : act_bwd(zf[j], act));
            NormVec<S16>::put(dz, off, d);
#pragma unroll
            for (int j = 0; j < V; ++j) p0[j] += d[j];
          }
        }
      }
      if (MODE != 3) {
#pragma unroll
        for (int j = 0; j < V; ++j) { s0[j] += (double)p0[j]; if (NS == 2) s1[j] += (double)p1[j]; }
      }
    }
  }
  if (MODE == 3) return;
  double t0[V], t1[V];
  const bool fold = (CW & (CW - 1)) == 0;
  if (fold) {
    for (int m = CW; m < 64; m <<= 1) {
#pragma unroll
      for (int j = 0; j < V; ++j) {
        s0[j] += __shfl_xor(s0[j], m, 64);
        if (NS == 2) s1[j] += __shfl_xor(s1[j], m, 64);
      }
    }
    const int lane = tid & 63, wv = tid >> 6;
    if (lane < CW) {
#pragma unroll
      for (int j = 0; j < V; ++j) {
        red[(wv * CW + lane) * 2 * V + j] = s0[j];
        red[(wv * CW + lane) * 2 * V + V + j] = s1[j];
      }
    }
    __syncthreads();
    if (tid < CW) {
#pragma unroll
      for (int j = 0; j < V; ++j) { t0[j] = red[tid * 2 * V + j]; t1[j] = red[tid * 2 * V + V + j]; }
#pragma unroll
      for (int w = 1; w < 4; ++w)
#pragma unroll
        for (int j = 0; j < V; ++j) {
          t0[j] += red[(w * CW + tid) * 2 * V + j];
          t1[j] += red[(w * CW + tid) * 2 * V + V + j];
        }
    }
  } else {
#pragma unroll
    for (int j = 0; j < V; ++j) {
      red[tid * 2 * V + j] = s0[j];
      red[tid * 2 * V + V + j] = s1[j];
    }
    __syncthreads();
    if (r0 == 0 && c4 < C4) {
#pragma unroll
      for (int j = 0; j < V; ++j) { t0[j] = 0.0; t1[j] = 0.0; }
      for (int k = 0; k < rpi; ++k) {
#pragma unroll
        for (int j = 0; j < V; ++j) {
          t0[j] += red[(k * CW + cq) * 2 * V + j];
          t1[j] += red[(k * CW + cq) * 2 * V + V + j];
        }
      }
    }
  }
  if (r0 == 0 && c4 < C4) {
    if (t.kind == NORM_TAIL_NONE) {
#pragma unroll
      for (int j = 0; j < V; ++j) {
        pout[c4 * V + j] = t0[j];
        if (NS == 2) pout[g.C + c4 * V + j] = t1[j];
      }
    } else {
#pragma unroll
      for (int j = 0; j < V; ++j) {
        norm_st_sc1(pout + c4 * V + j, t0[j]);
        if (NS == 2) norm_st_sc1(pout + g.C + c4 * V + j, t1[j]);
      }
    }
  }
  if (t.kind == NORM_TAIL_NONE) return;

  if (!norm_arrive(t.ctr + n * g.slices + slice, (unsigned)g.chunks, tid, &s_flag)) return;
  const int SC = CW * V;
  const int c_lo = slice * SC;
  const int nout = NS * SC;
  int KG = 256 / nout;
  {
    const int o = tid % nout, kg = tid / nout;
    const int sidx = o / SC, c = c_lo + o % SC;
    double acc = 0.0;
    if (kg < KG && c < g.C) {
      const double* src = part + ((size_t)n * g.chunks * 3 + sidx) * g.C + c;
      const size_t kstride = (size_t)3 * g.C;
#pragma unroll 8
      for (int k = kg; k < g.chunks; k += KG) acc += src[k * kstride];
    }
    red[tid] = acc;
    __syncthreads();
    if (kg == 0) {
      double tot = 0.0;
      for (int j = 0; j < KG; ++j) tot += red[j * nout + o];
      red[256 + o] = tot;
      if (c < g.C) norm_st_sc1(t.nc + ((size_t)sidx * g.N + n) * g.C + c, tot);
    }
  }
  unsigned* const ctr2 = t.ctr + g.N * g.slices;
  if (t.kind == NORM_TAIL_PS_FWD) {
    if (!norm_arrive(ctr2 + n, (unsigned)g.slices, tid, &s_flag)) return;
    const int groups = (t.norm == MSEG_NORM_GN) ? 8 : g.C;
    const int cg = g.C / groups;
    const double* S = t.nc + (size_t)n * g.C;
    const double* Q = t.nc + ((size_t)g.N + n) * g.C;
    for (int base = 0; base < groups; base += 128) {
      const int grp = base + tid;
      if (tid < 128 && grp < groups) {
        double sm = 0.0, q = 0.0;
        for (int k = 0; k < cg; ++k) { sm += S[grp * cg + k]; q += Q[grp * cg + k]; }
        const double cnt = (double)cg * g.HW;
        const double mean = sm / cnt;
        double var = q / cnt - mean * mean;
        if (var < 0.0) var = 0.0;
        const double rstd = 1.0 / sqrt(var + (double)t.eps);
        red[tid] = mean; red[128 + tid] = rstd;
        t.mean_out[n * groups + grp] = (float)mean;
        t.rstd_out[n * groups + grp] = (float)rstd;
      }
      __syncthreads();
      const int c_end = (base + 128 < groups ? base + 128 : groups) * cg;
      for (int c = base * cg + tid; c < c_end; c += 256) {
        const int gl = c / cg - base;
        const double mean = red[gl], rstd = red[128 + gl];
        const double ga = (t.norm == MSEG_NORM_GN && t.gamma) ? (double)t.gamma[c] : 1.0;
        const double be = (t.norm == MSEG_NORM_GN && t.beta) ? (double)t.beta[c] : 0.0;
        t.scale[(size_t)n * g.C + c] = (float)(ga * rstd);
        t.shift[(size_t)n * g.C + c] = (float)(be - mean * ga * rstd);
      }
      __syncthreads();
    }
    return;
  }
  if (!norm_arrive(ctr2 + slice, (unsigned)g.N, tid, &s_flag)) return;
  {
    const int o = tid % nout;
    const int sidx = o / SC, c = c_lo + o % SC;
    if (tid < nout) {
      double sm = 0.0;
      if (c < g.C) {
        const double* src = t.nc + (size_t)sidx * g.N * g.C + c;
#pragma unroll 8
        for (int i = 0; i < g.N; ++i) sm += src[(size_t)i * g.C];
      }
      red[o] = sm;
    }
    __syncthreads();
    const int c2 = c_lo + tid;
    if (tid < SC && c2 < g.C) {
      const double a0 = red[tid], b0 = NS == 2 ? red[SC + tid] : 0.0;
      const double cnt = (double)g.N * g.HW;
      if (t.kind == NORM_TAIL_COLSUM) {
        t.colsum[c2] = (float)a0;
      } else if (t.kind == NORM_TAIL_BN_FWD) {
// ... 153 lines not shown
    return;
  }
  const int groups = (norm == MSEG_NORM_GN) ? 8 : g.C;
  const int cg = g.C / groups;
  const int total = g.N * g.C;
  for (int i = first; i < total; i += stride) {
    const int c = i % g.C, n = i / g.C;
    const int grp = c / cg;
    const double mu = mean[n * groups + grp], r = rstd[n * groups + grp];
    double m1 = 0.0, m2 = 0.0;
    for (int k = 0; k < cg; ++k) {
      const int cc = grp * cg + k;
      const double ga = (norm == MSEG_NORM_GN && gamma) ? (double)gamma[cc] : 1.0;
      const double s1 = S1[(size_t)n * g.C + cc], s2 = S2[(size_t)n * g.C + cc];
      m1 += ga * s1;
      m2 += ga * r * (s2 - mu * s1);
    }
    const double cnt = (double)cg * g.HW;
    m1 /= cnt; m2 /= cnt;
    const double gac = (norm == MSEG_NORM_GN && gamma) ? (double)gamma[c] : 1.0;
    k1[i] = (float)(gac * r);
    k2[i] = (float)(-r * r * m2);
    k3[i] = (float)(-r * m1 + r * r * m2 * mu);
  }
  if (norm == MSEG_NORM_GN && dgamma) {
    for (int c = first; c < g.C; c += stride) {
      const int grp = c / cg;
      double dg = 0.0, db = 0.0;
      for (int n = 0; n < g.N; ++n) {
        const double mu = mean[n * groups + grp], r = rstd[n * groups + grp];
        const double s1 = S1[(size_t)n * g.C + c], s2 = S2[(size_t)n * g.C + c];
        dg += r * (s2 - mu * s1);
        db += s1;
      }
      dgamma[c] = (float)dg;
      if (dbeta) dbeta[c] = (float)db;
    }
  }
}

__global__ void norm_bwd_finalize_kernel(const double* __restrict__ nc, NormGeom g, int norm,
                                         const float* __restrict__ gamma, const float* __restrict__ mean,
                                         const float* __restrict__ rstd, float* __restrict__ k1,
                                         float* __restrict__ k2, float* __restrict__ k3, float* __restrict__ dgamma,
                                         float* __restrict__ dbeta) {
  norm_bwd_finalize_body(nc, g, norm, gamma, mean, rstd, k1, k2, k3, dgamma, dbeta, blockIdx.x * blockDim.x + threadIdx.x,
                         gridDim.x * blockDim.x);
}

__device__ __forceinline__ void norm_colsum_body(const double* __restrict__ nc, const NormGeom& g, float* __restrict__ out,
                                                 int first, int stride) {
  for (int c = first; c < g.C; c += stride) {
    double s = 0.0;
#pragma unroll 8
    for (int n = 0; n < g.N; ++n) s += nc[(size_t)n * g.C + c];
    out[c] = (float)s;
  }
}
__global__ void norm_colsum_kernel(const double* __restrict__ nc, NormGeom g, float* __restrict__ out) {
  norm_colsum_body(nc, g, out, blockIdx.x * blockDim.x + threadIdx.x, gridDim.x * blockDim.x);
}

__global__ __launch_bounds__(256) void norm_reduce_finish_kernel(const double* __restrict__ part, double* __restrict__ nc,
                                                                 NormGeom g, int ns, const NormTail t) {
  __shared__ double red[8][32];
  __shared__ int s_flag;
  norm_reduce_chunks_body(part, nc, g, ns, true, red);
  if (!norm_arrive(t.ctr + NORM_CTR_MAX - 1, gridDim.x, threadIdx.x, &s_flag)) return;
  if (t.kind == NORM_TAIL_BN_FWD)
    norm_fwd_finalize_body(nc, g, MSEG_NORM_BN, t.gamma, t.beta, t.eps, t.scale, t.shift, t.mean_out, t.rstd_out, t.running_mean,
                           t.running_var, t.momentum, 0.0, threadIdx.x, 256);
  else if (t.kind == NORM_TAIL_BN_BWD)
    norm_bwd_finalize_body(nc, g, MSEG_NORM_BN, t.gamma, t.mean, t.rstd, t.k1, t.k2, t.k3, t.dgamma, t.dbeta, threadIdx.x, 256);
  else
    norm_colsum_body(nc, g, t.colsum, threadIdx.x, 256);
}

#define NORM_FB_CH 4
#define NORM_FB_NB 64
__global__ __launch_bounds__(1024) void norm_bn_finish_kernel(const double* __restrict__ part, double* __restrict__ nc,
                                                             NormGeom g, int ns, const NormTail t) {
  __shared__ double red[NORM_FB_NB][8][NORM_FB_CH];
  __shared__ double tn[NORM_FB_NB][NORM_FB_CH];
  __shared__ double tot[3][NORM_FB_CH];
  const int tid = threadIdx.x;
  const int cl = tid & 3, kg = (tid >> 2) & 7, nl = tid >> 5, nlanes = (int)blockDim.x >> 5;
  const int c = blockIdx.x * NORM_FB_CH + cl;
  const bool cok = c < g.C;
  for (int sidx = 0; sidx < ns; ++sidx) {
    double run = 0.0;
    for (int n0 = 0; n0 < g.N; n0 += NORM_FB_NB) {
      const int nb = g.N - n0 < NORM_FB_NB ? g.N - n0 : NORM_FB_NB;
#pragma unroll 2
      for (int nn = nl; nn < nb; nn += nlanes) {
        double acc = 0.0;
        if (cok) {
          const double* src = part + (((size_t)(n0 + nn) * g.chunks) * 3 + sidx) * g.C + c;
          const size_t kstride = (size_t)3 * g.C;
#pragma unroll 4
          for (int k = kg; k < g.chunks; k += 8) acc += src[k * kstride];
        }
        red[nn][kg][cl] = acc;
      }
      __syncthreads();
      {
        const int nn = tid >> 2;
        if (nn < nb) {
          double s8 = 0.0;
#pragma unroll
          for (int j = 0; j < 8; ++j) s8 += red[nn][j][cl];
          tn[nn][cl] = s8;
          if (cok) nc[((size_t)sidx * g.N + n0 + nn) * g.C + c] = s8;
        }
      }
      __syncthreads();
      if (tid < NORM_FB_CH)
        for (int nn = 0; nn < nb; ++nn) run += tn[nn][tid];
      __syncthreads();
    }
    if (tid < NORM_FB_CH) tot[sidx][tid] = run;
  }
  if (tid >= NORM_FB_CH || !cok) return;
  const double a0 = tot[0][tid], b0 = ns > 1 ? tot[1][tid] : 0.0;
  if (t.kind == NORM_TAIL_BN_FWD) {
    const double cnt = (double)g.N * g.HW;
    const double mean = a0 / cnt;
    double var = b0 / cnt - mean * mean;
    if (var < 0.0) var = 0.0;
    const double rstd = 1.0 / sqrt(var + (double)t.eps);
    const double ga = t.gamma ? (double)t.gamma[c] : 1.0, be = t.beta ? (double)t.beta[c] : 0.0;
    t.scale[c] = (float)(ga * rstd);
    t.shift[c] = (float)(be - mean * ga * rstd);
    t.mean_out[c] = (float)mean;
    t.rstd_out[c] = (float)rstd;
    if (t.running_mean) {
      const double unb = cnt > 1.0 ? var * cnt / (cnt - 1.0) : var;
      t.running_mean[c] = (float)((1.0 - (double)t.momentum) * t.running_mean[c] + (double)t.momentum * mean);
      t.running_var[c] = (float)((1.0 - (double)t.momentum) * t.running_var[c] + (double)t.momentum * unb);
    }
  } else if (t.kind == NORM_TAIL_BN_BWD) {
    const double cnt = (double)g.N * g.HW;
    const double mu = t.mean[c], r = t.rstd[c], ga = t.gamma ? (double)t.gamma[c] : 1.0;
    const double sx = r * (b0 - mu * a0);
    const double m1 = ga * a0 / cnt, m2 = ga * sx / cnt;
    t.k1[c] = (float)(ga * r);
    t.k2[c] = (float)(-r * r * m2);
    t.k3[c] = (float)(-r * m1 + r * r * m2 * mu);
    if (t.dgamma) t.dgamma[c] = (float)sx;
    if (t.dbeta) t.dbeta[c] = (float)a0;
  } else {
    t.colsum[c] = (float)a0;
  }
}

__global__ void bn_eval_coeffs_kernel(const float* __restrict__ gamma, const float* __restrict__ beta,
                                      const float* __restrict__ rm, const float* __restrict__ rv, float eps, int C,
                                      float* __restrict__ scale, float* __restrict__ shift) {
  const int c = blockIdx.x * blockDim.x + threadIdx.x;
  if (c >= C) return;
  const float inv = 1.0f / sqrtf(rv[c] + eps);
  const float sc = (gamma ? gamma[c] : 1.f) * inv;
  scale[c] = sc;
  shift[c] = (beta ? beta[c] : 0.f) - rm[c] * sc;
}

static inline unsigned nblocks(size_t n, unsigned cap = 1024u) {
  size_t b = (n + 255) / 256;
  if (b < 1) b = 1;
  return (unsigned)(b > cap ? cap : b);
}

#define NORM_PASS_A(MODE_, S16_, ...)                                                                                \
  do {                                                                                                               \
    if (aio_) hipLaunchKernelGGL((norm_pass_kernel<MODE_, S16_, true>), dim3(g.chunks, N, g.slices), dim3(256), 0, st, __VA_ARGS__); \
    else hipLaunchKernelGGL((norm_pass_kernel<MODE_, S16_, false>), dim3(g.chunks, N, g.slices), dim3(256), 0, st, __VA_ARGS__);     \
  } while (0)
#define NORM_PASS(MODE_, AIO_, ...)                                                                                  \
  do {                                                                                                               \
    auto aio_ = (AIO_);                                                                                              \
    if (st_ == MSEG_ST_BF16) NORM_PASS_A(MODE_, true, __VA_ARGS__);                                                  \
    else NORM_PASS_A(MODE_, false, __VA_ARGS__);                                                                     \
  } while (0)

static int g_norm_finish = -1;
extern "C" int mseg_norm_set_finish(int on) {
  g_norm_finish = on < 0 ? -1 : (on > 2 ? 2 : on);
  return MSEG_OK;
}
static int norm_finish_mode() {
  if (g_norm_finish < 0) {
    const char* e = getenv("MSEG_NORM_FINISH");
    g_norm_finish = e ? atoi(e) : 2;
    if (g_norm_finish < 0 || g_norm_finish > 2) g_norm_finish = 2;
  }
  return g_norm_finish;
}
static bool norm_finish_fits(int C) { return norm_finish_mode() == 2 || (norm_finish_mode() == 1 && C <= 256); }
static void norm_launch_finish(const double* part, double* nc, const NormGeom& g, int ns, const NormTail& tf, int N, int C,
                               hipStream_t st) {
  if (norm_finish_mode() == 2)
    hipLaunchKernelGGL(norm_bn_finish_kernel, dim3((unsigned)((C + NORM_FB_CH - 1) / NORM_FB_CH)), dim3(N > 8 ? 1024 : 256), 0,
                       st, part, nc, g, ns, tf);
  else
    hipLaunchKernelGGL(norm_reduce_finish_kernel, dim3(nblocks((size_t)ns * N * C * 8, 4096u)), dim3(256), 0, st, part, nc, g,
                       ns, tf);
}
static int g_norm_tails = -1;
extern "C" int mseg_norm_set_tails(int on) {
  g_norm_tails = on ? 1 : 0;
  return MSEG_OK;
}
static bool norm_tails_fit(const NormGeom& g) {
  if (g_norm_tails < 0) {
    const char* e = getenv("MSEG_NORM_TAILS");
    g_norm_tails = e ? (atoi(e) != 0) : 0;
  }
  return g_norm_tails && (long long)g.N * g.slices + (g.N > g.slices ? g.N : g.slices) <= NORM_CTR_MAX;
}

extern "C" int mseg_norm_stats(const void* z, int N, int HW, int C, int st_, int act, int norm, const float* gamma,
                               const float* beta, float eps, float* scale, float* shift, float* mean, float* rstd,
                               float* running_mean, float* running_var, float momentum, void* act_out, void* ws,
                               void* stream) {
  if (!z || !scale || !shift || !mean || !rstd || !ws || N <= 0 || HW <= 0 || C <= 0 || (C & 3)) return MSEG_EINVAL;
  if (st_ != MSEG_ST_F32 && st_ != MSEG_ST_BF16) return MSEG_EINVAL;
  if (st_ == MSEG_ST_BF16 && (C & 7)) return MSEG_EINVAL;
  if (norm == MSEG_NORM_GN && (C % 8)) return MSEG_EINVAL;
  if (norm < 0 || norm > 2) return MSEG_EINVAL;
  if ((running_mean == nullptr) != (running_var == nullptr)) return MSEG_EINVAL;
  hipStream_t st = (hipStream_t)stream;
  NormGeom g = norm_geom(N, HW, C, norm_vec(st_));
  double* part = (double*)((char*)ws + NORM_CTR_BYTES);
// ... 67 lines not shown
  return MSEG_OK;
}

extern "C" int mseg_activation(const void* z, int N, int HW, int C, int st_, int act, void* act_out, void* stream) {
  if (!z || !act_out || N <= 0 || HW <= 0 || C <= 0 || (C & 3)) return MSEG_EINVAL;
  if ((st_ != MSEG_ST_F32 && st_ != MSEG_ST_BF16) || (st_ == MSEG_ST_BF16 && (C & 7))) return MSEG_EINVAL;
  hipStream_t st = (hipStream_t)stream;
  NormGeom g = norm_geom(N, HW, C, norm_vec(st_));
  NormTail t = {};
  NORM_PASS(3, act_out, z, (const void*)nullptr, (void*)nullptr, (const float*)nullptr, (const float*)nullptr,
            (const float*)nullptr, 0, g, act, (double*)nullptr, aio_, t);
  MSEG_LAUNCH_CHECK();
  return MSEG_OK;
}

extern "C" int mseg_bn_eval_coeffs(const float* gamma, const float* beta, const float* running_mean,
                                   const float* running_var, float eps, int C, float* scale, float* shift,
                                   void* stream) {
  if (!running_mean || !running_var || !scale || !shift || C <= 0) return MSEG_EINVAL;
  hipLaunchKernelGGL(bn_eval_coeffs_kernel, dim3((C + 255) / 256), dim3(256), 0, (hipStream_t)stream, gamma, beta,
                     running_mean, running_var, eps, C, scale, shift);
  MSEG_LAUNCH_CHECK();
  return MSEG_OK;
}

extern "C" int mseg_norm_bwd(const void* gy, const void* z, int N, int HW, int C, int st_, int act, int norm,
                             const float* gamma, const float* mean, const float* rstd, void* dz, float* dgamma,
                             float* dbeta, float* dbias, const void* act_in, void* ws, void* stream) {
  if (!gy || !z || !mean || !rstd || !dz || !ws || N <= 0 || HW <= 0 || C <= 0 || (C & 3)) return MSEG_EINVAL;
  if ((st_ != MSEG_ST_F32 && st_ != MSEG_ST_BF16) || (st_ == MSEG_ST_BF16 && (C & 7))) return MSEG_EINVAL;
  if (norm < 0 || norm > 2) return MSEG_EINVAL;
  if (norm == MSEG_NORM_GN && (C % 8)) return MSEG_EINVAL;
  hipStream_t st = (hipStream_t)stream;
  NormGeom g = norm_geom(N, HW, C, norm_vec(st_));
  double* part = (double*)((char*)ws + NORM_CTR_BYTES);
  double* nc = part + (size_t)N * g.chunks * 3 * C;
  float* k1 = (float*)(nc + (size_t)3 * N * C);
  float* k2 = k1 + (size_t)N * C;
  float* k3 = k2 + (size_t)N * C;
  const int kss = (norm == MSEG_NORM_BN) ? 0 : C;
  const bool tails = norm_tails_fit(g);
  NormTail t = {};
  t.kind = (tails && norm == MSEG_NORM_BN) ? NORM_TAIL_BN_BWD : NORM_TAIL_NONE;
  t.norm = norm; t.ctr = (unsigned*)ws; t.nc = nc; t.gamma = gamma; t.mean = mean; t.rstd = rstd;
  t.k1 = k1; t.k2 = k2; t.k3 = k3; t.dgamma = dgamma; t.dbeta = dbeta;
  NORM_PASS(1, const_cast<void*>(act_in), z, gy, (void*)nullptr, (const float*)nullptr, (const float*)nullptr,
            (const float*)nullptr, 0, g, act, part, aio_, t);
  MSEG_LAUNCH_CHECK();
  if (t.kind == NORM_TAIL_NONE && norm == MSEG_NORM_BN && norm_finish_fits(C)) {
    NormTail tf = t;
    tf.kind = NORM_TAIL_BN_BWD;
    norm_launch_finish((const double*)part, nc, g, 2, tf, N, C, st);
    MSEG_LAUNCH_CHECK();
  } else if (t.kind == NORM_TAIL_NONE) {
    hipLaunchKernelGGL(norm_reduce_chunks_kernel, dim3(nblocks((size_t)2 * N * C * 8, 4096u)), dim3(256), 0, st,
                       (const double*)part, nc, g, 2);
    MSEG_LAUNCH_CHECK();
    hipLaunchKernelGGL(norm_bwd_finalize_kernel, dim3(nblocks(norm == MSEG_NORM_BN ? C : (size_t)N * C)), dim3(256), 0,
                       st, (const double*)nc, g, norm, gamma, mean, rstd, k1, k2, k3, dgamma, dbeta);
    MSEG_LAUNCH_CHECK();
  }
  double* part2 = part;
  NormTail t2 = {};
  t2.kind = (tails && dbias) ? NORM_TAIL_COLSUM : NORM_TAIL_NONE;
  t2.norm = norm; t2.ctr = (unsigned*)ws; t2.nc = nc; t2.colsum = dbias;
  NORM_PASS(2, const_cast<void*>(act_in), z, gy, dz, (const float*)k1, (const float*)k2, (const float*)k3, kss, g, act,
            part2, aio_, t2);
  MSEG_LAUNCH_CHECK();
  if (dbias && t2.kind == NORM_TAIL_NONE && norm_finish_fits(C)) {
    NormTail tf = t2;
    tf.kind = NORM_TAIL_COLSUM;
    norm_launch_finish((const double*)part2, nc, g, 1, tf, N, C, st);
    MSEG_LAUNCH_CHECK();
  } else if (dbias && t2.kind == NORM_TAIL_NONE) {
    hipLaunchKernelGGL(norm_reduce_chunks_kernel, dim3(nblocks((size_t)N * C * 8, 4096u)), dim3(256), 0, st,
                       (const double*)part2, nc, g, 1);
    MSEG_LAUNCH_CHECK();
    hipLaunchKernelGGL(norm_colsum_kernel, dim3(nblocks(C)), dim3(256), 0, st, (const double*)nc, g, dbias);
    MSEG_LAUNCH_CHECK();
  }
  return MSEG_OK;
}

__global__ void maxpool_fwd_kernel(const MsegSrc s, int N, int H, int W, float* __restrict__ out) {
  const int Ho = H >> 1, Wo = W >> 1, C4 = s.C >> 2;
  const size_t total = (size_t)N * Ho * Wo * C4;
  for (size_t i = (size_t)blockIdx.x * blockDim.x + threadIdx.x; i < total; i += (size_t)gridDim.x * blockDim.x) {
    const int c = (int)(i % C4) * 4;
    size_t r = i / C4;
    const int x = (int)(r % Wo); r /= Wo;
    const int y = (int)(r % Ho);
    const int n = (int)(r / Ho);
    float4 best;
#pragma unroll
    for (int k = 0; k < 4; ++k) {
      const size_t pix = ((size_t)n * H + 2 * y + (k >> 1)) * W + 2 * x + (k & 1);
      float4 v = *reinterpret_cast<const float4*>(s.ptr + pix * s.C + c);
      v = src_transform4(v, s, n, c);
      if (k == 0) best = v;
      else { best.x = v.x > best.x ? v.x : best.x; best.y = v.y > best.y ? v.y : best.y;
             best.z = v.z > best.z ? v.z : best.z; best.w = v.w > best.w ? v.w : best.w; }
    }
    *reinterpret_cast<float4*>(out + i * 4) = best;
  }
}

__global__ void maxpool_bwd_kernel(const MsegSrc s, int N, int H, int W, const float* __restrict__ gout,
                                   float* __restrict__ gin, int accumulate) {
  const int Ho = H >> 1, Wo = W >> 1, C4 = s.C >> 2;
  const size_t total = (size_t)N * Ho * Wo * C4;
  for (size_t i = (size_t)blockIdx.x * blockDim.x + threadIdx.x; i < total; i += (size_t)gridDim.x * blockDim.x) {
    const int c = (int)(i % C4) * 4;
    size_t r = i / C4;
    const int x = (int)(r % Wo); r /= Wo;
    const int y = (int)(r % Ho);
    const int n = (int)(r / Ho);
    float4 v[4];
    size_t off[4];
#pragma unroll
    for (int k = 0; k < 4; ++k) {
      const size_t pix = ((size_t)n * H + 2 * y + (k >> 1)) * W + 2 * x + (k & 1);
      off[k] = pix * s.C + c;
      v[k] = src_transform4(*reinterpret_cast<const float4*>(s.ptr + off[k]), s, n, c);
    }
    const float4 g = *reinterpret_cast<const float4*>(gout + i * 4);
    int ax = 0, ay = 0, az = 0, aw = 0;
#pragma unroll
    for (int k = 1; k < 4; ++k) {
      if (v[k].x > v[ax].x) ax = k;
      if (v[k].y > v[ay].y) ay = k;
      if (v[k].z > v[az].z) az = k;
      if (v[k].w > v[aw].w) aw = k;
    }
#pragma unroll
    for (int k = 0; k < 4; ++k) {
      float4 o = make_float4(ax == k ? g.x : 0.f, ay == k ? g.y : 0.f, az == k ? g.z : 0.f, aw == k ? g.w : 0.f);
      if (accumulate) {
        const float4 old = *reinterpret_cast<const float4*>(gin + off[k]);
        o.x += old.x; o.y += old.y; o.z += old.z; o.w += old.w;
      }
      *reinterpret_cast<float4*>(gin + off[k]) = o;
    }
  }
}

extern "C" int mseg_maxpool2x2_fwd(const MsegSrc* src, int N, int H, int W, float* out, void* stream) {
  if (!src || !src->ptr || !out || N <= 0 || H <= 0 || W <= 0 || (H & 1) || (W & 1) || (src->C & 3)) return MSEG_EINVAL;
  if (src->dtype != MSEG_ST_F32) return MSEG_EINVAL;
  const size_t total = (size_t)N * (H / 2) * (W / 2) * (src->C / 4);
  hipLaunchKernelGGL(maxpool_fwd_kernel, dim3(nblocks(total, 8192u)), dim3(256), 0, (hipStream_t)stream, *src, N, H, W, out);
  MSEG_LAUNCH_CHECK();
  return MSEG_OK;
}

extern "C" int mseg_maxpool2x2_bwd(const MsegSrc* src, int N, int H, int W, const float* gout, float* gin,
                                   int accumulate, void* stream) {
  if (!src || !src->ptr || !gout || !gin || N <= 0 || H <= 0 || W <= 0 || (H & 1) || (W & 1) || (src->C & 3))
    return MSEG_EINVAL;
  if (src->dtype != MSEG_ST_F32) return MSEG_EINVAL;
  const size_t total = (size_t)N * (H / 2) * (W / 2) * (src->C / 4);
  hipLaunchKernelGGL(maxpool_bwd_kernel, dim3(nblocks(total, 8192u)), dim3(256), 0, (hipStream_t)stream, *src, N, H, W,
                     gout, gin, accumulate);
  MSEG_LAUNCH_CHECK();
  return MSEG_OK;
}
```

### microbeseg_amd/engine.py

```python
import ctypes as C
import os

import torch

from . import _lib
from ._lib import (ACT, NORM, MODE_CONV, MODE_TCONV, EPI_PLAIN, EPI_SCATTER2X2, MORDER_LINEAR, MORDER_PARITY,
                   ST_F32, ST_BF16, MsegSrc, MsegIgemm, MsegWgrad, MsegKernelInfo, check)

BN_EPS = 1e-5
BN_MOMENTUM = 0.1


def _ptr(t):
    return None if t is None else t.data_ptr()


def _stream():
    return torch.cuda.current_stream().cuda_stream


def _pad4(c):
    return (c + 3) // 4 * 4


# ... 246 lines not shown
    def mark_fresh(self):
        self.version, self.src_ptr = self.param._version, self.param.data_ptr()

    def refresh(self):
        lib = _lib.load()
        T, R, rpad, Cc, kpad, st, sr, sc = self.job
        src = self.param.detach()
        check(lib.mseg_pack_weight(src.data_ptr(), self.t.data_ptr(), T, R, rpad, Cc, kpad, st, sr, sc, _stream()),
              "pack_weight")
        if self._t16 is not None:
            check(lib.mseg_f32_to_bf16(self.t.data_ptr(), self._t16.data_ptr(), self.t.numel(), _stream()), "f32_to_bf16")
        self.mark_fresh()

    def bf16(self):
        if self._t16 is None:
            if self.merge:
                self._t16 = torch.zeros(self.t.numel(), dtype=torch.bfloat16, device=self.t.device)
            else:
                self._t16 = torch.empty(self.t.numel(), dtype=torch.bfloat16, device=self.t.device)
            check(_lib.load().mseg_f32_to_bf16(self.t.data_ptr(), self._t16.data_ptr(), self.t.numel(), _stream()),
                  "f32_to_bf16")
        return self._t16


def pack_weight(param, T, R, Cc, st, sr, sc, merge_taps=False, kind=None):
    if kind is None:
        e = PackedW(param, T, R, Cc, st, sr, sc, merge_taps)
        e.refresh()
        return e
    packs = param.__dict__.get("_mseg_packs")
    if packs is None:
        packs = param.__dict__["_mseg_packs"] = {}
    e = packs.get(kind)
    if e is None:
        e = packs[kind] = PackedW(param, T, R, Cc, st, sr, sc, merge_taps)
    if e.stale():
        e.refresh()
    return e


_pack_tables = {}


def repack_all(params):
    entries = []
    for p in params:
        packs = p.__dict__.get("_mseg_packs")
        if packs:
            entries += [e for _, e in sorted(packs.items())]
    if not entries:
        return 0
    key = tuple((id(e), e.param.data_ptr(), e.t.data_ptr(), 0 if e._t16 is None else e._t16.data_ptr(), e.job)
                for e in entries)
    tab = _pack_tables.get(key)
    if tab is None:
        _pack_tables.clear()
        jobs = (_lib.MsegPackJob * len(entries))()
        nblk = 0
        for j, e in zip(jobs, entries):
            T, R, rpad, Cc, kpad, st, sr, sc = e.job
            j.src, j.dst = e.param.data_ptr(), e.t.data_ptr()
            j.dst16 = None if e._t16 is None else e._t16.data_ptr()
            j.T, j.R, j.Rpad, j.C, j.Cpad, j.st, j.sr, j.sc = T, R, rpad, Cc, kpad, st, sr, sc
            j.first_block = nblk
            nblk += _lib.load().mseg_pack_job_blocks(T, rpad, kpad)
        raw = torch.frombuffer(bytearray(bytes(jobs)), dtype=torch.uint8)
        tab = (raw.to(entries[0].t.device), len(entries), nblk)
        _pack_tables[key] = tab
    check(_lib.load().mseg_pack_weights_multi(tab[0].data_ptr(), tab[1], tab[2], _stream()), "pack_weights_multi")
    for e in entries:
        e.mark_fresh()
    return len(entries)


def mark_packs_fresh(params):
    for p in params:
        packs = p.__dict__.get("_mseg_packs")
        if packs:
            for e in packs.values():
                e.mark_fresh()


class KernelChoice:
    __slots__ = ("name", "bf16", "launches", "grid", "block", "workspace", "stats_rows")

    def __init__(self, info):
        self.name = info.name.decode()
        self.bf16 = info.precision == 1
        self.launches, self.grid, self.block, self.workspace = info.launches, info.grid, info.block, info.workspace
        self.stats_rows = info.stats_rows

    def __repr__(self):
        return f"KernelChoice({self.name!r}, bf16={self.bf16}, grid={self.grid})"


def _fill_igemm(p, srcs, kpad, npad, NB, Hi, Wi, Ho, Wo, KH, KW, stride, pad, mode, Ngemm, ld0, acc0, ld1, acc1, split, epi,
                Cq, morder):
    for i, s in enumerate(srcs):
        p.src[i] = s
    p.nsrc = len(srcs)
    p.Cin = sum(s.C for s in srcs)
    p.Kpad, p.Npad = kpad, npad
    p.NB, p.Hi, p.Wi, p.Ho, p.Wo = NB, Hi, Wi, Ho, Wo
    p.KH, p.KW, p.stride, p.pad, p.mode, p.morder = KH, KW, stride, pad, mode, morder
    p.Ngemm, p.epi = Ngemm, epi
    p.split = Ngemm if split is None else split
    p.ld0, p.ld1, p.acc0, p.acc1, p.Cq = ld0, ld1, acc0, acc1, Cq


def _query(fn, p):
    info = MsegKernelInfo()
    rc = fn(C.byref(p), C.byref(info))
    return KernelChoice(info) if rc == 0 else None


def igemm_query(srcs, kpad, npad, NB, Hi, Wi, Ho, Wo, KH, KW, stride, pad, mode, Ngemm, ld0, acc0=0, ld1=0, acc1=0,
                split=None, epi=EPI_PLAIN, Cq=0, morder=MORDER_LINEAR, precision=None, dst_dtype=ST_F32, bias=True):
    p = MsegIgemm()
    _fill_igemm(p, srcs, kpad, npad, NB, Hi, Wi, Ho, Wo, KH, KW, stride, pad, mode, Ngemm, ld0, acc0, ld1, acc1, split, epi, Cq,
                morder)
    p.w = p.dst0 = _DUMMY
    p.dst1 = _DUMMY if (split is not None and split < Ngemm) else None
    p.bias = _DUMMY if bias else None
    p.precision = 1 if (precision or _precision) == "bf16" else 0
    p.dst_dtype = dst_dtype
    return _query(_lib.load().mseg_igemm_query, p)


_bf16_ok_cache = {}


def _igemm_bf16_ok(p):
    key = (p.nsrc, tuple((p.src[i].C, p.src[i].act, bool(p.src[i].scale), p.src[i].ss != 0, p.src[i].dtype)
                         for i in range(p.nsrc)), p.Kpad, p.Npad, p.NB, p.Hi, p.Wi, p.Ho, p.Wo, p.KH, p.KW, p.stride, p.pad,
           p.mode, p.morder, p.Ngemm, p.epi, p.split, p.ld0, p.ld1, p.acc0, p.acc1, p.Cq, p.dst_dtype, bool(p.bias))
    ok = _bf16_ok_cache.get(key)
    if ok is None:
        p.precision = 1
        ok = _bf16_ok_cache[key] = _query(_lib.load().mseg_igemm_query, p) is not None
    return ok


_conv_stats = os.environ.get("MSEG_CONV_STATS", "0") == "1"


def set_conv_stats(flag):
    global _conv_stats
    old, _conv_stats = _conv_stats, bool(flag)
    return old


def igemm(srcs, w, bias, NB, Hi, Wi, Ho, Wo, KH, KW, stride, pad, mode, Ngemm, dst0, ld0, acc0=0,
          dst1=None, ld1=0, acc1=0, split=None, epi=EPI_PLAIN, Cq=0, morder=MORDER_LINEAR, real_cin=None,
          precision=None, stats=None):
    lib = _lib.load()
    p = MsegIgemm()
    _fill_igemm(p, srcs, w.Kpad, w.Npad, NB, Hi, Wi, Ho, Wo, KH, KW, stride, pad, mode, Ngemm, ld0, acc0, ld1, acc1, split, epi,
                Cq, morder)
    p.w = w.t.data_ptr()
    p.dst_dtype = _st(dst0)
    p.bias = _ptr(bias)
    p.dst0 = dst0.data_ptr()
    p.dst1 = _ptr(dst1)
    bf16 = (precision or _precision) == "bf16" and _igemm_bf16_ok(p)
    if bf16:
        p.w = w.bf16().data_ptr()
    p.precision = 1 if bf16 else 0
    need = lib.mseg_igemm_workspace_bytes(C.byref(p))
    if need:
        key = (dst0.device, _stream())
        buf = _splitk_ws.get(key)
        if buf is None or buf.numel() < need:
            buf = torch.empty(need, dtype=torch.uint8, device=dst0.device)
            _splitk_ws[key] = buf
        p.ws, p.ws_bytes = buf.data_ptr(), buf.numel()
    taken = None
    if stats is not None and bf16 and _conv_stats:
        p.stats, p.stats_act = _DUMMY, stats[0]
        choice = _query(lib.mseg_igemm_query, p)
        rows = choice.stats_rows if choice else 0
        if rows > 0:
            part = stats[1].get("convstats", rows * 2 * Ngemm * 4)
            p.stats = part.data_ptr()
            taken = (part, rows)
        else:
            p.stats = None
    if _timer is None:
        check(lib.mseg_igemm(C.byref(p), _stream()), "igemm")
        return taken
    flops = 2.0 * NB * Ho * Wo * Ngemm * (p.Cin if real_cin is None else real_cin) * KH * KW
    if mode == MODE_TCONV:
        flops /= stride * stride
    choice = _query(lib.mseg_igemm_query, p)
    e0, e1 = _timer.bracket(choice.name if choice else "igemm?", flops)
    e0.record()
    check(lib.mseg_igemm(C.byref(p), _stream()), "igemm")
    e1.record()
    return taken


def _fill_wgrad(p, P, Qs, NB, Hp, Wp, Hq, Wq, KH, KW, stride, pad, nch_store):
    p.P = P
    for i, s in enumerate(Qs):
        p.Q[i] = s
    p.nq = len(Qs)
    p.Nch = sum(s.C for s in Qs)
    p.Nch_store = p.Nch if nch_store is None else nch_store
    p.NB, p.Hp, p.Wp, p.Hq, p.Wq = NB, Hp, Wp, Hq, Wq
    p.KH, p.KW, p.stride, p.pad = KH, KW, stride, pad
    p.splits = 0


def wgrad_query(P, Qs, NB, Hp, Wp, Hq, Wq, KH, KW, stride, pad, nch_store=None, precision=None):
    p = MsegWgrad()
    _fill_wgrad(p, P, Qs, NB, Hp, Wp, Hq, Wq, KH, KW, stride, pad, nch_store)
    p.precision = 1 if (precision or _precision) == "bf16" else 0
    p.dst = p.ws = _DUMMY
    p.phase = 1
    return _query(_lib.load().mseg_wgrad_query, p)


def _wgrad_bf16_ok(p):
    key = ((p.P.C, p.P.act, bool(p.P.scale), p.P.ss != 0, p.P.dtype),
           tuple((p.Q[i].C, p.Q[i].act, bool(p.Q[i].scale), p.Q[i].ss != 0, p.Q[i].dtype) for i in range(p.nq)),
           p.Nch_store, p.NB, p.Hp, p.Wp, p.Hq, p.Wq, p.KH, p.KW, p.stride, p.pad)
    ok = _bf16_ok_cache.get(key)
    if ok is None:
        q = MsegWgrad()
        C.memmove(C.byref(q), C.byref(p), C.sizeof(MsegWgrad))
        q.precision, q.phase = 1, 1
        q.dst = q.ws = _DUMMY
        ok = _bf16_ok_cache[key] = _query(_lib.load().mseg_wgrad_query, q) is not None
    return ok


def wgrad(P, Qs, dst, NB, Hp, Wp, Hq, Wq, KH, KW, stride, pad, ws, nch_store=None, precision=None):
    lib = _lib.load()
    p = MsegWgrad()
    _fill_wgrad(p, P, Qs, NB, Hp, Wp, Hq, Wq, KH, KW, stride, pad, nch_store)
    bf16 = (precision or _precision) == "bf16" and _wgrad_bf16_ok(p)
    p.precision = 1 if bf16 else 0
    p.dst = dst.data_ptr()
    need = lib.mseg_wgrad_workspace_bytes(C.byref(p))
    if need == 0:
        raise RuntimeError("libmseg_hip wgrad: unsupported shape")
    p.ws = ws.get("wgrad", need).data_ptr()
    if _timer is None:
        check(lib.mseg_wgrad(C.byref(p), _stream()), "wgrad")
        return
    flops = 2.0 * NB * Hp * Wp * P.C * p.Nch_store * KH * KW
    p.phase = 1
    choice = _query(lib.mseg_wgrad_query, p)
    e0, e1 = _timer.bracket(choice.name if choice else "wgrad?", flops)
    e0.record()
    check(lib.mseg_wgrad(C.byref(p), _stream()), "wgrad")
    e1.record()
    p.phase = 2
    check(lib.mseg_wgrad(C.byref(p), _stream()), "wgrad_reduce")


_stats_epoch = 0


def note_training_step():
    global _stats_epoch
    _stats_epoch += 1


def norm_stats(node, norm, gamma, beta, running_mean, running_var, training, ws, conv_part=None):
    lib = _lib.load()
    dev = node.z.device
    node.norm = norm
    N, HW, Cc = node.N, node.H * node.W, node.C
    expensive = node.act not in (ACT["none"], ACT["relu"])
    if expensive:
        node.a = torch.empty_like(node.z)
    if norm == NORM["bn"]:
        node.ss = 0
        if not training:
            key = (_stats_epoch,) + tuple((t.data_ptr(), t._version) if t is not None else None
                                          for t in (gamma, beta, running_mean, running_var))
            cached = running_mean.__dict__.get("_mseg_eval")
            if cached is None or cached[0] != key:
                scale = torch.empty(Cc, dtype=torch.float32, device=dev)
                shift = torch.empty(Cc, dtype=torch.float32, device=dev)
                check(lib.mseg_bn_eval_coeffs(_ptr(gamma), _ptr(beta), running_mean.data_ptr(), running_var.data_ptr(),
                                              BN_EPS, Cc, scale.data_ptr(), shift.data_ptr(), _stream()), "bn_eval_coeffs")
                cached = (key, scale, shift)
                running_mean.__dict__["_mseg_eval"] = cached
            node.scale, node.shift = cached[1], cached[2]
            if expensive:
                check(lib.mseg_activation(node.z.data_ptr(), N, HW, Cc, _st(node.z), node.act, node.a.data_ptr(),
                                          _stream()), "activation")
            return
        node.scale = torch.empty(Cc, dtype=torch.float32, device=dev)
        node.shift = torch.empty(Cc, dtype=torch.float32, device=dev)
        node.mean = torch.empty(Cc, dtype=torch.float32, device=dev)
        node.rstd = torch.empty(Cc, dtype=torch.float32, device=dev)
    else:
        node.ss = Cc
        node.scale = torch.empty(N * Cc, dtype=torch.float32, device=dev)
        node.shift = torch.empty(N * Cc, dtype=torch.float32, device=dev)
        ng = 8 if norm == NORM["gn"] else Cc
        node.mean = torch.empty(N * ng, dtype=torch.float32, device=dev)
        node.rstd = torch.empty(N * ng, dtype=torch.float32, device=dev)
        running_mean = running_var = None
    w = ws.get("norm", lib.mseg_norm_workspace_bytes(N, HW, Cc), zero=True)
    if conv_part is not None and norm == NORM["bn"] and not expensive:
        check(lib.mseg_norm_stats_from_conv(conv_part[0].data_ptr(), conv_part[1], Cc, N * HW, _ptr(gamma), _ptr(beta),
                                            BN_EPS, node.scale.data_ptr(), node.shift.data_ptr(), node.mean.data_ptr(),
                                            node.rstd.data_ptr(), _ptr(running_mean), _ptr(running_var), BN_MOMENTUM,
                                            w.data_ptr(), _stream()), "norm_stats_from_conv")
    else:
        check(lib.mseg_norm_stats(node.z.data_ptr(), N, HW, Cc, _st(node.z), node.act, norm, _ptr(gamma), _ptr(beta),
                                  BN_EPS, node.scale.data_ptr(), node.shift.data_ptr(), node.mean.data_ptr(),
                                  node.rstd.data_ptr(), _ptr(running_mean), _ptr(running_var), BN_MOMENTUM,
                                  _ptr(node.a), w.data_ptr(), _stream()), "norm_stats")
    if running_mean is not None:
        torch.autograd.graph.increment_version((running_mean, running_var))
        note_training_step()


def norm_bwd(node, gy, gamma, dgamma, dbeta, dbias, ws):
    lib = _lib.load()
    N, HW, Cc = node.N, node.H * node.W, node.C
    w = ws.get("norm", lib.mseg_norm_workspace_bytes(N, HW, Cc), zero=True)
    check(lib.mseg_norm_bwd(gy.data_ptr(), node.z.data_ptr(), N, HW, Cc, _st(node.z), node.act, node.norm, _ptr(gamma),
                            node.mean.data_ptr(), node.rstd.data_ptr(), gy.data_ptr(), _ptr(dgamma), _ptr(dbeta),
                            _ptr(dbias), _ptr(node.a), w.data_ptr(), _stream()), "norm_bwd")
    return gy


class ConvSpec:

    def __init__(self, kind, conv, norm_mod, act, norm):
        self.kind = kind
        self.conv = conv
        self.norm_mod = norm_mod
        self.act = ACT[act]
        self.norm = NORM[norm]

    def params(self):
        ps = [self.conv.weight, self.conv.bias]
        if self.norm in (NORM["bn"], NORM["gn"]):
            ps += [self.norm_mod.weight, self.norm_mod.bias]
        return ps


class HeadSpec:
    def __init__(self, conv):
        self.conv = conv

    def params(self):
        return [self.conv.weight, self.conv.bias]


class NetSpec:
    def __init__(self, ch_in, enc, decoders, pool_method):
        self.ch_in = ch_in
        self.enc = enc
        self.decoders = decoders
        self.pool_method = pool_method

    def layers(self):
        out = []
        for e in self.enc:
            out += [e["c1"], e["c2"]]
            if e["pool"] is not None and e["pool"] != "max":
                out.append(e["pool"])
        for d in self.decoders:
            for lv in d["levels"]:
                out += [lv["up"], lv["c1"], lv["c2"]]
            out.append(d["head"])
        return out

    def params(self):
        ps = []
        for l in self.layers():
            ps += l.params()
        return ps


class Tape:

    def __init__(self):
        self.nodes = []
        self.heads = []
        self.x4 = None


class RawFrame:
    PIX = {torch.uint8: 0, torch.uint16: 1, torch.int16: 1}

    def __init__(self, raw, pad_top=0, pad_left=0):
        if raw.dim() != 2 or raw.dtype not in self.PIX or not raw.is_cuda or not raw.is_contiguous():
            raise RuntimeError("RawFrame: a contiguous 2-D uint8 / uint16 CUDA tensor expected")
        self.raw, self.pad_top, self.pad_left = raw, int(pad_top), int(pad_left)
        self.minmax = torch.empty(2, dtype=torch.int32, device=raw.device)
        self.H, self.W = raw.shape[0] + self.pad_top, raw.shape[1] + self.pad_left
        check(_lib.load().mseg_frame_minmax(raw.data_ptr(), self.PIX[raw.dtype], raw.numel(), self.minmax.data_ptr(),
                                            _stream()), "frame_minmax")

    @property
    def device(self):
        return self.raw.device

    def args(self):
        return (self.raw.data_ptr(), self.PIX[self.raw.dtype], self.raw.shape[0], self.raw.shape[1], self.pad_top,
                self.pad_left, self.minmax.data_ptr())

    def normalized(self):
        out = torch.empty((1, 1, self.H, self.W), dtype=torch.float32, device=self.raw.device)
        check(_lib.load().mseg_frame_normalize(*self.args(), out.data_ptr(), _stream()), "frame_normalize")
# ... 133 lines not shown
        tape.x4 = xin
    st = torch.bfloat16 if (_precision == "bf16" and _bf16_storage and
                            bf16_storage_ok(spec, N, cin, H, W, keep_tape)) else torch.float32

    cur = xin
    skips = []
    for i, e in enumerate(spec.enc):
        cur = _run_conv(e["c1"], [cur], training, ws, tape, first_layer_cin=cin if i == 0 else None, st=st)
        cur = _run_conv(e["c2"], [cur], training, ws, tape, st=st)
        if e["pool"] is not None:
            skips.append(cur)
            if e["pool"] == "max":
                cur = _run_maxpool(cur, tape)
            else:
                cur = _run_conv(e["pool"], [cur], training, ws, tape, st=st)
    bottom = cur
    outs = []
    dec_stream = None
    if _decoder_overlap and _precision == "bf16" and len(spec.decoders) > 1 and dev.type == "cuda" and \
            not torch.cuda.is_current_stream_capturing():
        dec_stream = _decoder_side_stream(dev)
        main = torch.cuda.current_stream(dev)

    def run_decoder(d, ws_):
        cur = bottom
        for lv, skip in zip(d["levels"], reversed(skips)):
            up = _run_conv(lv["up"], [cur], training, ws_, tape, st=st)
            cur = _run_conv(lv["c1"], [up, skip], training, ws_, tape, st=st)
            cur = _run_conv(lv["c2"], [cur], training, ws_, tape, st=st)
        hc = d["head"].conv
        co = hc.weight.shape[0]
        out = torch.empty((N, co, H, W), dtype=torch.float32, device=dev)
        s = cur.src()
        check(lib.mseg_head_fwd(C.byref(s), N, H * W, hc.weight.detach().data_ptr(), hc.bias.detach().data_ptr(), co,
                                out.data_ptr(), _stream()), "head_fwd")
        if tape is not None:
            tape.heads.append((d["head"], cur))
        return out

    for k, d in enumerate(spec.decoders):
        if dec_stream is not None and k == len(spec.decoders) - 1:
            dec_stream.wait_stream(main)
            with torch.cuda.stream(dec_stream):
                outs.append(run_decoder(d, _SideWs(ws, "@dec")))
        else:
            outs.append(run_decoder(d, ws))
    if dec_stream is not None:
        main.wait_stream(dec_stream)
    if _nbt_pending:
        torch._foreach_add_(_nbt_pending, 1)
        del _nbt_pending[:]
    return outs, tape


def _accumulate_target(node, shape_like):
    if node.grad is None:
        node.grad = torch.empty_like(node.z)
        return node.grad, 0
    return node.grad, 1


def _grad_buf(param, direct):
    d = param.__dict__
    if d.get("_mseg_grad_direct") and d.get("_mseg_grad_fresh") and param.grad is not None:
        d["_mseg_grad_fresh"] = False
        direct.add(id(param))
        return param.grad
    return torch.empty_like(param)


_wgrad_overlap = os.environ.get("MSEG_WGRAD_OVERLAP", "1") != "0"
_side_streams = {}


def set_wgrad_overlap(flag):
    global _wgrad_overlap
    _wgrad_overlap = bool(flag)


def get_wgrad_overlap():
    return _wgrad_overlap


_overlap_in_capture = os.environ.get("MSEG_OVERLAP_IN_CAPTURE", "0") == "1"


_decoder_overlap = os.environ.get("MSEG_DECODER_OVERLAP", "0") == "1"


def set_decoder_overlap(flag):
    global _decoder_overlap
    _decoder_overlap = bool(flag)


def get_decoder_overlap():
    return _decoder_overlap


def _decoder_side_stream(dev):
    s = _side_streams.get((dev, "dec"))
    if s is None:
        s = _side_streams[(dev, "dec")] = torch.cuda.Stream(device=dev)
    return s


_SIDE_HOLD_BYTES = 16 << 30


def _wgrad_side_stream(dev):
    s = _side_streams.get(dev)
    if s is None:
        s = _side_streams[dev] = torch.cuda.Stream(device=dev, priority=0)
    return s


def backward(spec, tape, grad_outs, ws, on_grads=None, direct=None):
    lib = _lib.load()
    grads = {}
    if direct is None:
        direct = set()
    dev = tape.nodes[0].z.device
    side = None
    if _wgrad_overlap and _precision == "bf16" and on_grads is None and dev.type == "cuda" and \
            (_overlap_in_capture or not torch.cuda.is_current_stream_capturing()):
        side = _wgrad_side_stream(dev)
        main = torch.cuda.current_stream(dev)
        side.wait_stream(main)

    held, held_bytes = [], [0]

    def on_side(dz, fn):
        if side is None:
            return fn(ws)
        ev = torch.cuda.Event()
        ev.record(main)
        with torch.cuda.stream(side):
            side.wait_event(ev)
            fn(_SideWs(ws))
        held.append(dz)
        held_bytes[0] += dz.numel() * dz.element_size()
        if held_bytes[0] > _SIDE_HOLD_BYTES:
            main.wait_stream(side)
            held.clear()
            held_bytes[0] = 0

    for (head, node), go in zip(tape.heads, grad_outs):
        hc = head.conv
        co = hc.weight.shape[0]
        if go is None:
            go = torch.zeros((node.N, co, node.H, node.W), dtype=torch.float32, device=node.z.device)
        go = go.contiguous().float()
        gy = torch.empty_like(node.z)
        dW = _grad_buf(hc.weight, direct)
        db = _grad_buf(hc.bias, direct)
        w = ws.get("head", lib.mseg_head_bwd_workspace_bytes(node.N, node.H * node.W, node.C, co))
        s = node.src()
        check(lib.mseg_head_bwd(C.byref(s), node.N, node.H * node.W, hc.weight.detach().data_ptr(), co,
                                go.data_ptr(), gy.data_ptr(), _st(gy), dW.data_ptr(), db.data_ptr(), w.data_ptr(),
                                _stream()), "head_bwd")
        assert node.grad is None
        node.grad = gy
        grads[id(hc.weight)] = dW
        grads[id(hc.bias)] = db
        if on_grads is not None:
            on_grads([dW, db])

    for node in reversed(tape.nodes):
        sp = node.layer
        gy = node.grad
        node.grad = None
        if gy is None:
            raise RuntimeError("internal: node without gradient")
        if sp is _MaxPoolMarker:
            i0 = node.inputs[0]
            tgt, acc = _accumulate_target(i0, None)
            s = i0.src()
            check(lib.mseg_maxpool2x2_bwd(C.byref(s), i0.N, i0.H, i0.W, gy.data_ptr(), tgt.data_ptr(), acc, _stream()),
                  "maxpool_bwd")
            continue
        conv = sp.conv
        nm = sp.norm_mod
        has_affine = sp.norm in (NORM["bn"], NORM["gn"])
        dgamma = _grad_buf(nm.weight, direct) if has_affine else None
        dbeta = _grad_buf(nm.bias, direct) if has_affine else None
        dbias = _grad_buf(conv.bias, direct)
        dz = norm_bwd(node, gy, nm.weight.detach() if has_affine else None, dgamma, dbeta, dbias, ws)
        if has_affine:
            grads[id(nm.weight)] = dgamma
            grads[id(nm.bias)] = dbeta
        grads[id(conv.bias)] = dbias
        wt = conv.weight.detach()
        dW = _grad_buf(conv.weight, direct)
        ins = node.inputs
        i0 = ins[0]
        N = node.N
        if sp.kind == "up":
            cin, cout = wt.shape[0], wt.shape[1]
            on_side(dz, lambda w_, i0=i0, dz=dz, dW=dW, cout=cout, node=node: wgrad(
                i0.src(), [plain_src(dz, cout)], dW, N, i0.H, i0.W, node.H, node.W, 2, 2, 2, 0, w_))
            wp = pack_weight(conv.weight, 4, cin, cout, 1, cout * 4, 4, kind="dgrad")
            tgt, acc = _accumulate_target(i0, None)
            igemm([plain_src(dz, cout)], wp, None, N, node.H, node.W, i0.H, i0.W, 2, 2, 2, 0, MODE_CONV, cin,
                  tgt, cin, acc0=acc)
        else:
            cout, cin = wt.shape[0], wt.shape[1]
            stride = 2 if sp.kind == "pool" else 1
            is_first = i0 is tape.x4
            if is_first and cin == 1 and _first_layer_ok(cin, cout, stride):
                w1 = ws.get("first_wgrad", lib.mseg_first_wgrad_workspace_bytes(N, node.H, node.W, cout))
                check(lib.mseg_first_wgrad(i0.z.data_ptr(), dz.data_ptr(), _st(dz), N, node.H, node.W, cout, dW.data_ptr(),
                                           w1.data_ptr(), _stream()), "first_wgrad")
            else:
                on_side(dz, lambda w_, dz=dz, ins=ins, dW=dW, cout=cout, node=node, i0=i0, stride=stride, cin=cin,
                        is_first=is_first: wgrad(plain_src(dz, cout), [n.src() for n in ins], dW, N, node.H, node.W, i0.H,
                                                 i0.W, 3, 3, stride, 1, w_, nch_store=cin if is_first else None))
            if not is_first:
                wp = pack_weight(conv.weight, 9, cin, cout, 1, 9, cin * 9, kind="dgrad")
                morder = MORDER_PARITY if stride == 2 else MORDER_LINEAR
                if len(ins) == 1:
                    tgt, acc = _accumulate_target(i0, None)
                    igemm([plain_src(dz, cout)], wp, None, N, node.H, node.W, i0.H, i0.W, 3, 3, stride, 1,
                          MODE_TCONV, cin, tgt, cin, acc0=acc, morder=morder)
                else:
                    i1 = ins[1]
                    t0, a0 = _accumulate_target(i0, None)
                    t1, a1 = _accumulate_target(i1, None)
                    igemm([plain_src(dz, cout)], wp, None, N, node.H, node.W, i0.H, i0.W, 3, 3, stride, 1,
                          MODE_TCONV, cin, t0, i0.C, acc0=a0, dst1=t1, ld1=i1.C, acc1=a1,
                          split=i0.C, morder=morder)
        grads[id(conv.weight)] = dW
        if on_grads is not None:
            on_grads([dW, dbias, dgamma, dbeta])
        del dz, gy
    if side is not None:
        main.wait_stream(side)
        held.clear()
    return grads


class _SideWs:

    def __init__(self, ws, tag="@side"):
        self.ws, self.tag = ws, tag

    def get(self, name, nbytes, zero=False):
        return self.ws.get(name + self.tag, nbytes, zero)


class _NetFunction(torch.autograd.Function):
    @staticmethod
    def forward(ctx, module, x, *params):
        training = module.training
        outs, tape = forward(module._spec, x, training, True, module._workspace(x.device))
        ctx.module = module
        ctx.tape = tape
        ctx.nparams = len(params)
        return tuple(outs)

    @staticmethod
    def backward(ctx, *grad_outs):
        module = ctx.module
        tape = ctx.tape
        if tape is None:
            raise RuntimeError("backward through the HIP U-Net twice is not supported")
        ctx.tape = None
        factory = getattr(module, "_grad_sync_factory", None)
        sync = factory() if factory is not None else None
        direct = set()
        grads = backward(module._spec, tape, list(grad_outs), module._workspace(tape.nodes[0].z.device),
                         on_grads=sync.add if sync is not None else None, direct=direct)
        if sync is not None:
            sync.finish()
        plist = module._spec.params()
        return (None, None) + tuple(None if id(p) in direct else grads.get(id(p)) for p in plist)


def run_module(module, x):
    if isinstance(x, RawFrame):
        outs, _ = forward(module._spec, x, module.training, False, module._workspace(x.device))
        return tuple(outs)
    if not x.is_cuda:
        raise RuntimeError(
            "microbeseg_amd: the U-Net runs on the MI355X HIP path only (got a CPU tensor); there is deliberately "
            "no CPU fallback in the product path — use the oracle under oracle/ for CPU reference runs")
    _lib.load()
    x = x.contiguous().float()
    plist = module._spec.params()
    need_grad = torch.is_grad_enabled() and any(p.requires_grad for p in plist)
    if need_grad:
        return _NetFunction.apply(module, x, *plist)
    outs, _ = forward(module._spec, x, module.training, False, module._workspace(x.device))
    return tuple(outs)
```

Before: 243.4 crops/s.

## Fuse norm-backward dz application into dgrad implicit-GEMM halo load

Measured after the change: 245.3 crops/s, median of 6. Within noise of the previous version (+0.8%).

```diff
diff --git a/include/mseg_hip.h b/include/mseg_hip.h
--- a/include/mseg_hip.h
+++ b/include/mseg_hip.h
@@ -61,6 +61,13 @@
   float* stats;
   int32_t stats_act;
   int32_t reserved0;
+  const float* dz_z;
+  const float* dz_k1;
+  const float* dz_k2;
+  const float* dz_k3;
+  float* dz_out;
+  int32_t dz_kss;
+  int32_t dz_act;
 } MsegIgemm;
 
 int mseg_igemm(const MsegIgemm* p, void* stream);
@@ -72,7 +79,7 @@
   uint32_t grid, block;
   size_t workspace;
   int32_t stats_rows;
-  int32_t reserved0;
+  int32_t dz_on_load;
 } MsegKernelInfo;
 int mseg_igemm_query(const MsegIgemm* p, MsegKernelInfo* info);
 const char* mseg_last_kernel(void);
@@ -147,6 +154,11 @@
 int mseg_norm_bwd(const void* gy, const void* z, int N, int HW, int C, int st, int act, int norm, const float* gamma,
                   const float* mean, const float* rstd, void* dz, float* dgamma, float* dbeta, float* dbias,
                   const void* act_in , void* ws, void* stream);
+
+int mseg_norm_bwd_coeffs_supported(int st, int act, int norm);
+int mseg_norm_bwd_coeffs(const void* gy, const void* z, int N, int HW, int C, int st, int act, int norm, const float* gamma,
+                         const float* mean, const float* rstd, float* k1, float* k2, float* k3, float* dgamma,
+                         float* dbeta, float* dbias, void* ws, void* stream);
 
 int mseg_maxpool2x2_fwd(const MsegSrc* src, int N, int H, int W, float* out, void* stream);
 int mseg_maxpool2x2_bwd(const MsegSrc* src, int N, int H, int W, const float* gout, float* gin, int accumulate,
diff --git a/microbeseg_amd/_lib.py b/microbeseg_amd/_lib.py
--- a/microbeseg_amd/_lib.py
+++ b/microbeseg_amd/_lib.py
@@ -33,7 +33,9 @@
                 ("Ngemm", C.c_int32), ("epi", C.c_int32), ("split", C.c_int32), ("ld0", C.c_int32),
                 ("ld1", C.c_int32), ("acc0", C.c_int32), ("acc1", C.c_int32), ("Cq", C.c_int32),
                 ("precision", C.c_int32), ("dst_dtype", C.c_int32), ("ws", C.c_void_p), ("ws_bytes", C.c_size_t),
-                ("stats", C.c_void_p), ("stats_act", C.c_int32), ("reserved0", C.c_int32)]
+                ("stats", C.c_void_p), ("stats_act", C.c_int32), ("reserved0", C.c_int32),
+                ("dz_z", C.c_void_p), ("dz_k1", C.c_void_p), ("dz_k2", C.c_void_p), ("dz_k3", C.c_void_p),
+                ("dz_out", C.c_void_p), ("dz_kss", C.c_int32), ("dz_act", C.c_int32)]
 
 
 class MsegWgrad(C.Structure):
@@ -46,7 +48,7 @@
 
 class MsegKernelInfo(C.Structure):
     _fields_ = [("name", C.c_char * 120), ("precision", C.c_int32), ("launches", C.c_int32), ("grid", C.c_uint32),
-                ("block", C.c_uint32), ("workspace", C.c_size_t), ("stats_rows", C.c_int32), ("reserved0", C.c_int32)]
+                ("block", C.c_uint32), ("workspace", C.c_size_t), ("stats_rows", C.c_int32), ("dz_on_load", C.c_int32)]
 
 
 class MsegPackJob(C.Structure):
@@ -99,6 +101,8 @@
     "mseg_activation": (_I, [_P, _I, _I, _I, _I, _I, _P, _P]),
     "mseg_bn_eval_coeffs": (_I, [_P, _P, _P, _P, _F, _I, _P, _P, _P]),
     "mseg_norm_bwd": (_I, [_P, _P, _I, _I, _I, _I, _I, _I, _P, _P, _P, _P, _P, _P, _P, _P, _P, _P]),
+    "mseg_norm_bwd_coeffs_supported": (_I, [_I, _I, _I]),
+    "mseg_norm_bwd_coeffs": (_I, [_P, _P, _I, _I, _I, _I, _I, _I, _P, _P, _P, _P, _P, _P, _P, _P, _P, _P, _P]),
     "mseg_maxpool2x2_fwd": (_I, [C.POINTER(MsegSrc), _I, _I, _I, _P, _P]),
     "mseg_maxpool2x2_bwd": (_I, [C.POINTER(MsegSrc), _I, _I, _I, _P, _P, _I, _P]),
     "mseg_head_fwd": (_I, [C.POINTER(MsegSrc), _I, _I, _P, _P, _I, _P, _P]),
diff --git a/microbeseg_amd/csrc/api_misc.hip b/microbeseg_amd/csrc/api_misc.hip
--- a/microbeseg_amd/csrc/api_misc.hip
+++ b/microbeseg_amd/csrc/api_misc.hip
@@ -35,6 +35,7 @@
   g_call.workspace = workspace;
 }
 extern "C" void mseg_dispatch_note_stats(int rows) { g_call.stats_rows = rows; }
+extern "C" void mseg_dispatch_note_dz(int on) { g_call.dz_on_load = on; }
 extern "C" void mseg_note_launch(const char* kernel, unsigned grid, unsigned block, int aux) {
   g_call.launches += 1;
   if (aux || g_call.name[0]) return;
diff --git a/microbeseg_amd/csrc/common.h b/microbeseg_amd/csrc/common.h
--- a/microbeseg_amd/csrc/common.h
+++ b/microbeseg_amd/csrc/common.h
@@ -21,6 +21,7 @@
 extern "C" void mseg_dispatch_end(MsegKernelInfo* info);
 extern "C" void mseg_dispatch_note(int precision, size_t workspace);
 extern "C" void mseg_dispatch_note_stats(int rows);
+extern "C" void mseg_dispatch_note_dz(int on);
 #define MSEG_KL(K, grid_, block_, shmem_, st_, ...)                                              \
   do {                                                                                           \
     mseg_note_launch(#K, (unsigned)(grid_).x, (unsigned)(block_).x, 0);                          \
@@ -82,6 +83,10 @@
     case MSEG_ACT_MISH: return mish_bwd<false>(z);
     default: return 1.f;
   }
+}
+
+__device__ __forceinline__ float norm_bwd_apply(float k1, float gy, float k2, float a, float k3, float d) {
+  return __fmul_rn(__fadd_rn(fmaf(k1, gy, __fmul_rn(k2, a)), k3), d);
 }
 
 __device__ __forceinline__ float act_fwd_fast(float x, int act) {
diff --git a/microbeseg_amd/csrc/igemm.hip b/microbeseg_amd/csrc/igemm.hip
--- a/microbeseg_amd/csrc/igemm.hip
+++ b/microbeseg_amd/csrc/igemm.hip
@@ -463,9 +463,11 @@
   constexpr int HL = (HMAX * 8 + 511) / 512;
   constexpr int ASTAGE = HMAX * LDS_STRIDE;
   constexpr int BSTAGE = BN * LDS_STRIDE;
-  __shared__ __attribute__((aligned(16))) float lds[ASTAGE + 2 * BSTAGE];
+  constexpr bool DZ = (TR == 3);
+  __shared__ __attribute__((aligned(16))) float lds[ASTAGE + 2 * BSTAGE + (DZ ? 3 * KC : 0)];
   float* const Abuf = lds;
   float* const Bbuf = lds + ASTAGE;
+  float* const Kbuf = lds + ASTAGE + 2 * BSTAGE;
 
   const int tid = threadIdx.x, lane = tid & 63, wave = tid >> 6;
   const int wm = wave / Cfg::WN, wn = wave % Cfg::WN;
@@ -488,7 +490,7 @@
   const int oy0 = ty * TH, ox0 = tx * TW, n0 = tile_n * BN;
   const int band0 = oy0 > 0 ? oy0 - 1 : 0;
   const int band_rows = (oy0 + TH + 1 < H ? oy0 + TH + 1 : H) - band0;
-  const bool conv = p.mode == MSEG_MODE_CONV;
+  const bool conv = !DZ && p.mode == MSEG_MODE_CONV;
 
   int hpix[HL];
   unsigned hvalid = 0u;
@@ -500,6 +502,7 @@
     const bool ok = (hrow < HROWS) & (iy >= 0) & (iy < H) & (ix >= 0) & (ix < W);
     hpix[j] = (iy - band0) * W + ix;
     hvalid |= (unsigned)ok << j;
+    if (DZ) hvalid |= (unsigned)(ok & (hy >= 1) & (hy <= TH) & (hx >= 1) & (hx <= TW) & (tile_n == 0)) << (8 + j);
   }
   int abase[Cfg::MB];
 #pragma unroll
@@ -528,6 +531,12 @@
                                                                         band_rows * W * C1 * 4, 0x00020000);
   const __amdgpu_buffer_rsrc_t rsw = __builtin_amdgcn_make_buffer_rsrc(const_cast<float*>(p.w), 0,
                                                                         9 * p.Npad * p.Kpad * 4, 0x00020000);
+  const __amdgpu_buffer_rsrc_t rsz = __builtin_amdgcn_make_buffer_rsrc(
+      const_cast<float*>(DZ ? p.dz_z + ((size_t)img * H + band0) * W * p.src[0].C : base0), 0,
+      band_rows * W * p.src[0].C * 4, 0x00020000);
+  const __amdgpu_buffer_rsrc_t rsd = __builtin_amdgcn_make_buffer_rsrc(
+      DZ ? p.dz_out + ((size_t)img * H + band0) * W * p.src[0].C : const_cast<float*>(base0), 0,
+      band_rows * W * p.src[0].C * 4, 0x00020000);
   unsigned wvoff[Cfg::BROWS];
 #pragma unroll
   for (int i = 0; i < Cfg::BROWS; ++i) wvoff[i] = ((unsigned)(n0 + srow + 64 * i) * (unsigned)p.Kpad + scol * 4u) * 4u;
@@ -536,6 +545,50 @@
   unsigned hlive = 0u;
   int ract = 0;
   bool cur_s1 = false;
+
+  float4 tz;
+  auto dz_load = [&](int chunk, int j) {
+    const int c = chunk * KC + scol * 4;
+    const bool ok = (c < p.Cin) && ((hvalid >> j) & 1u);
+    const unsigned vo = ok ? (unsigned)hpix[j] * ((unsigned)C0 * 4u) + (unsigned)c * 4u : OOB;
+    const f32x4 v = __builtin_bit_cast(f32x4, __builtin_amdgcn_raw_buffer_load_b128(rs0, vo, 0, 0));
+    const f32x4 u = __builtin_bit_cast(f32x4, __builtin_amdgcn_raw_buffer_load_b128(rsz, vo, 0, 0));
+    rh[j] = make_float4(v[0], v[1], v[2], v[3]);
+    tz = make_float4(u[0], u[1], u[2], u[3]);
+  };
+  auto dz_apply = [&](int chunk, int j) {
+    const int c = chunk * KC + scol * 4;
+    const bool inb = c < p.Cin;
+    const bool ok = inb && ((hvalid >> j) & 1u);
+    const float4 k1 = *reinterpret_cast<const float4*>(Kbuf + scol * 4);
+    const float4 k2 = *reinterpret_cast<const float4*>(Kbuf + KC + scol * 4);
+    const float4 k3 = *reinterpret_cast<const float4*>(Kbuf + 2 * KC + scol * 4);
+    const int act = p.dz_act;
+    const float4 a = act_fwd4(tz, act);
+    const float live = ok ? 1.f : 0.f;
+    float4 g = rh[j];
+    g.x = norm_bwd_apply(k1.x, g.x, k2.x, a.x, k3.x, act == MSEG_ACT_RELU ? (tz.x > 0.f ? 1.f : 0.f) : live);
+    g.y = norm_bwd_apply(k1.y, g.y, k2.y, a.y, k3.y, act == MSEG_ACT_RELU ? (tz.y > 0.f ? 1.f : 0.f) : live);
+    g.z = norm_bwd_apply(k1.z, g.z, k2.z, a.z, k3.z, act == MSEG_ACT_RELU ? (tz.z > 0.f ? 1.f : 0.f) : live);
+    g.w = norm_bwd_apply(k1.w, g.w, k2.w, a.w, k3.w, act == MSEG_ACT_RELU ? (tz.w > 0.f ? 1.f : 0.f) : live);
+    rh[j] = g;
+    const bool st = inb && ((hvalid >> (8 + j)) & 1u);
+    const unsigned vo = st ? (unsigned)hpix[j] * ((unsigned)C0 * 4u) + (unsigned)c * 4u : OOB;
+    f32x4 o; o[0] = g.x; o[1] = g.y; o[2] = g.z; o[3] = g.w;
+    typedef unsigned u32x4 __attribute__((__vector_size__(16)));
+    __builtin_amdgcn_raw_buffer_store_b128(__builtin_bit_cast(u32x4, o), rsd, vo, 0, 0);
+  };
+  auto k_load = [&](int chunk) {
+    if (tid < 24) {
+      const int q = tid >> 3;
+      const float* kp = q == 0 ? p.dz_k1 : (q == 1 ? p.dz_k2 : p.dz_k3);
+      const int c = chunk * KC + scol * 4;
+      tz = *reinterpret_cast<const float4*>(kp + (size_t)img * (unsigned)p.dz_kss + (c < p.Cin ? c : 0));
+    }
+  };
+  auto k_store = [&]() {
+    if (tid < 24) *reinterpret_cast<float4*>(Kbuf + (tid >> 3) * KC + scol * 4) = tz;
+  };
 
   auto issue_halo = [&](int chunk) {
     const int c = chunk * KC + scol * 4;
@@ -552,7 +605,7 @@
                              : __builtin_bit_cast(f32x4, __builtin_amdgcn_raw_buffer_load_b128(rs0, vo, 0, 0));
       rh[j] = make_float4(v[0], v[1], v[2], v[3]);
     }
-    if (TR != 0) {
+    if (TR == 1 || TR == 2) {
       ract = s.act;
       const bool has_aff = s.scale != nullptr;
       const float* scp = has_aff ? s.scale : g_ident_scale;
@@ -571,7 +624,7 @@
       const int hrow = srow + 64 * j;
       if (hrow < HMAX) {
         float4 v = rh[j];
-        if (TR != 0) {
+        if (TR == 1 || TR == 2) {
           if (TR == 2) v = act_fwd4(v, ract);
           else { v.x = clamp_lo(v.x, lo); v.y = clamp_lo(v.y, lo); v.z = clamp_lo(v.z, lo); v.w = clamp_lo(v.w, lo); }
           const float m = ((hlive >> j) & 1u) ? 1.f : 0.f;
@@ -599,10 +652,23 @@
 
   const int c_begin = kz * chunks_per_split;
   const int c_end = (c_begin + chunks_per_split < nchunks) ? c_begin + chunks_per_split : nchunks;
-  issue_halo(c_begin);
+  if (DZ) {
+    k_load(c_begin);
+    k_store();
+    __syncthreads();
+#pragma unroll
+    for (int j = 0; j < HL; ++j) { dz_load(c_begin, j); dz_apply(c_begin, j); }
+  } else {
+    issue_halo(c_begin);
+  }
   issue_b(c_begin, 0);
   commit_halo(Abuf);
   commit_b(Bbuf);
+  if (DZ && c_begin + 1 < c_end) {
+    __syncthreads();
+    k_load(c_begin + 1);
+    k_store();
+  }
   __syncthreads();
 
   int bsel = 0;
@@ -610,6 +676,20 @@
     const float* As = Abuf;
     const bool more_chunks = chunk + 1 < c_end;
     for (int t = 0; t < 9; ++t) {
+      if (DZ) {
+        if (more_chunks) {
+#pragma unroll
+          for (int j = 0; j <= HL; ++j)
+            if (t == j) {
+              if (j > 0) dz_apply(chunk + 1, j - 1);
+              if (j < HL) dz_load(chunk + 1, j);
+            }
+        }
+        if (chunk + 2 < c_end) {
+          if (t == HL + 1) k_load(chunk + 2);
+          if (t == HL + 2) k_store();
+        }
+      } else
       if (t == 0 && more_chunks) issue_halo(chunk + 1);
       const bool last = (t == 8) && !more_chunks;
       issue_b(t == 8 ? (more_chunks ? chunk + 1 : chunk) : chunk, last ? 8 : (t == 8 ? 0 : t + 1));
@@ -2526,6 +2606,15 @@
     const int tr = plain ? 0 : (generic ? 2 : 1);
     int cps = 0;
     int ks = halo_ksplit(htiles, (p.Cin + KC - 1) / KC, &cps);
+    const bool want_dz = p.dz_out != nullptr;
+    if (want_dz) {
+      if (!(p.precision == MSEG_PREC_F32 && p.mode == MSEG_MODE_TCONV && p.nsrc == 1 && plain && !s16 && ks == 1 &&
+            p.dz_z && p.dz_k1 && p.dz_k2 && p.dz_k3 && (p.dz_kss & 3) == 0 && p.dz_kss >= 0 &&
+            (((uintptr_t)p.dz_k1 | (uintptr_t)p.dz_k2 | (uintptr_t)p.dz_k3 | (uintptr_t)p.dz_z | (uintptr_t)p.dz_out) & 15) == 0 &&
+            (p.dz_act == MSEG_ACT_NONE || p.dz_act == MSEG_ACT_RELU)))
+        return MSEG_EINVAL;
+      mseg_dispatch_note_dz(1);
+    }
     const size_t need = (size_t)ks * (size_t)M * (size_t)p.Ngemm * sizeof(float);
     if (ks > 1 && (!p.ws || p.ws_bytes < need || (p.Ngemm & 3) || (p.split & 3) || htiles * ks > 0x7fffffffLL)) {
       ks = 1;
@@ -2586,7 +2675,8 @@
     } else if (p.precision == MSEG_PREC_BF16) {
       if (wide) { if (tr == 0) MSEG_HALO16W4(0); else if (tr == 1) MSEG_HALO16W4(1); else MSEG_HALO16W4(2); }
       else      { if (tr == 0) MSEG_HALO16(64, 0); else if (tr == 1) MSEG_HALO16(64, 1); else MSEG_HALO16(64, 2); }
-    } else if (wide) { if (tr == 0) MSEG_HALO(128, 0); else if (tr == 1) MSEG_HALO(128, 1); else MSEG_HALO(128, 2); }
+    } else if (want_dz) { if (wide) MSEG_HALO(128, 3); else MSEG_HALO(64, 3); }
+    else if (wide) { if (tr == 0) MSEG_HALO(128, 0); else if (tr == 1) MSEG_HALO(128, 1); else MSEG_HALO(128, 2); }
     else      { if (tr == 0) MSEG_HALO(64, 0); else if (tr == 1) MSEG_HALO(64, 1); else MSEG_HALO(64, 2); }
 #undef MSEG_HALO
 #undef MSEG_HALO16
@@ -2603,6 +2693,7 @@
     }
     return MSEG_OK;
   }
+  if (p.dz_out) return MSEG_EINVAL;
   if (p.precision == MSEG_PREC_BF16 && s16 && g_c64p_on && p.epi == MSEG_EPI_SCATTER2X2 && p.KH == 1 && p.KW == 1 &&
       p.stride == 1 && p.pad == 0 && p.mode == MSEG_MODE_CONV && p.nsrc == 1 && p.Cin == 128 && p.Kpad == 128 &&
       p.Cq == 64 && p.Ngemm == 256 && !p.acc0 && (p.Wi % 32) == 0 && (((long long)p.Hi * p.Wi) % 128) == 0 &&
diff --git a/microbeseg_amd/csrc/norm.hip b/microbeseg_amd/csrc/norm.hip
--- a/microbeseg_amd/csrc/norm.hip
+++ b/microbeseg_amd/csrc/norm.hip
@@ -33,7 +33,8 @@
   if (N <= 0 || HW <= 0 || C <= 0) return 0;
   NormGeom g4 = norm_geom(N, HW, C, 4), g8 = norm_geom(N, HW, C, 8);
   const int chunks = g4.chunks > g8.chunks ? g4.chunks : g8.chunks;
-  return NORM_CTR_BYTES + ((size_t)N * chunks * 3 * C + (size_t)3 * N * C + (size_t)2 * N * C + (size_t)32 * C) * sizeof(double);
+  return NORM_CTR_BYTES + ((size_t)N * chunks * 3 * C + (size_t)3 * N * C + (size_t)2 * N * C + (size_t)32 * C +
+                           (size_t)N * chunks * 2 * C) * sizeof(double);
 }
 
 template <bool S16>
@@ -115,9 +116,63 @@
   float *scale, *shift, *mean_out, *rstd_out, *running_mean, *running_var;
   const float *mean, *rstd;
   float *k1, *k2, *k3, *dgamma, *dbeta, *colsum;
+  double* xpart;
+  float* dbias;
 };
 
-template <int MODE, bool S16, bool AIO>
+template <int V>
+__device__ __forceinline__ void norm_fold_pair(double (&s0)[V], double (&s1)[V], double* red, int tid, int CW, int rpi,
+                                               int cq, double (&t0)[V], double (&t1)[V]) {
+  if ((CW & (CW - 1)) == 0) {
+    for (int m = CW; m < 64; m <<= 1) {
+#pragma unroll
+      for (int j = 0; j < V; ++j) {
+        s0[j] += __shfl_xor(s0[j], m, 64);
+        s1[j] += __shfl_xor(s1[j], m, 64);
+      }
+    }
+    const int lane = tid & 63, wv = tid >> 6;
+    if (lane < CW) {
+#pragma unroll
+      for (int j = 0; j < V; ++j) {
+        red[(wv * CW + lane) * 2 * V + j] = s0[j];
+        red[(wv * CW + lane) * 2 * V + V + j] = s1[j];
+      }
+    }
+    __syncthreads();
+    if (tid < CW) {
+#pragma unroll
+      for (int j = 0; j < V; ++j) { t0[j] = red[tid * 2 * V + j]; t1[j] = red[tid * 2 * V + V + j]; }
+#pragma unroll
+      for (int w = 1; w < 4; ++w)
+#pragma unroll
+        for (int j = 0; j < V; ++j) {
+          t0[j] += red[(w * CW + tid) * 2 * V + j];
+          t1[j] += red[(w * CW + tid) * 2 * V + V + j];
+        }
+    }
+  } else {
+#pragma unroll
+    for (int j = 0; j < V; ++j) {
+      red[tid * 2 * V + j] = s0[j];
+      red[tid * 2 * V + V + j] = s1[j];
+    }
+    __syncthreads();
+    if (tid < CW) {
+#pragma unroll
+      for (int j = 0; j < V; ++j) { t0[j] = 0.0; t1[j] = 0.0; }
+      for (int k = 0; k < rpi; ++k) {
+#pragma unroll
+        for (int j = 0; j < V; ++j) {
+          t0[j] += red[(k * CW + cq) * 2 * V + j];
+          t1[j] += red[(k * CW + cq) * 2 * V + V + j];
+        }
+      }
+    }
+  }
+}
+
+template <int MODE, bool S16, bool AIO, bool XS = false>
 __global__ __launch_bounds__(256) void norm_pass_kernel(const void* __restrict__ z, const void* __restrict__ gy,
                                                         void* __restrict__ dz, const float* __restrict__ k1,
                                                         const float* __restrict__ k2, const float* __restrict__ k3,
@@ -140,8 +195,13 @@
   const int c4 = slice * CW + cq;
   const bool active = (c4 < C4) && (r0 < rpi);
   double s0[V], s1[V];
+  double x0[V], x1[V], x2[V];
 #pragma unroll
   for (int j = 0; j < V; ++j) { s0[j] = 0.0; s1[j] = 0.0; }
+  if (XS) {
+#pragma unroll
+    for (int j = 0; j < V; ++j) { x0[j] = 0.0; x1[j] = 0.0; x2[j] = 0.0; }
+  }
   if (active) {
     const int c = c4 * V;
     float a1[V], a2[V], a3[V];
@@ -156,8 +216,13 @@
       NormVec<S16> zv[U], gv[U], av[U];
       bool ok[U];
       float p0[V], p1[V];
+      float q0[V], q1[V], q2[V];
 #pragma unroll
       for (int j = 0; j < V; ++j) { p0[j] = 0.f; p1[j] = 0.f; }
+      if (XS) {
+#pragma unroll
+        for (int j = 0; j < V; ++j) { q0[j] = 0.f; q1[j] = 0.f; q2[j] = 0.f; }
+      }
 #pragma unroll
       for (int u = 0; u < U; ++u) {
         const int ru = r + u * rpi;
@@ -211,11 +276,18 @@
           if (MODE == 1) {
 #pragma unroll
             for (int j = 0; j < V; ++j) { p0[j] += gf[j]; p1[j] = fmaf(gf[j], a4[j], p1[j]); }
+            if (XS) {
+#pragma unroll
+              for (int j = 0; j < V; ++j) {
+                const float d = act_bwd(zf[j], act);
+                q0[j] += d; q1[j] = fmaf(gf[j], d, q1[j]); q2[j] = fmaf(a4[j], d, q2[j]);
+              }
+            }
           } else {
             float d[V];
 #pragma unroll
             for (int j = 0; j < V; ++j)
-              d[j] = (a1[j] * gf[j] + a2[j] * a4[j] + a3[j]) * (S16 ? act_bwd_fast(zf[j], act) : act_bwd(zf[j], act));
+              d[j] = norm_bwd_apply(a1[j], gf[j], a2[j], a4[j], a3[j], S16 ? act_bwd_fast(zf[j], act) : act_bwd(zf[j], act));
             NormVec<S16>::put(dz, off, d);
 #pragma unroll
             for (int j = 0; j < V; ++j) p0[j] += d[j];
@@ -225,6 +297,10 @@
       if (MODE != 3) {
 #pragma unroll
         for (int j = 0; j < V; ++j) { s0[j] += (double)p0[j]; if (NS == 2) s1[j] += (double)p1[j]; }
+      }
+      if (XS) {
+#pragma unroll
+        for (int j = 0; j < V; ++j) { x0[j] += (double)q0[j]; x1[j] += (double)q1[j]; x2[j] += (double)q2[j]; }
       }
     }
   }
@@ -292,6 +368,25 @@
         if (NS == 2) norm_st_sc1(pout + g.C + c4 * V + j, t1[j]);
       }
     }
+  }
+  if (XS) {
+    double* const xpout = t.xpart + ((size_t)n * g.chunks + chunk) * 2 * g.C;
+    double u0[V], u1[V];
+    __syncthreads();
+    norm_fold_pair<V>(x1, x2, red, tid, CW, rpi, cq, u0, u1);
+    if (r0 == 0 && c4 < C4) {
+#pragma unroll
+      for (int j = 0; j < V; ++j) { xpout[c4 * V + j] = u0[j]; xpout[g.C + c4 * V + j] = u1[j]; }
+    }
+    __syncthreads();
+#pragma unroll
+    for (int j = 0; j < V; ++j) x1[j] = 0.0;
+    norm_fold_pair<V>(x0, x1, red, tid, CW, rpi, cq, u0, u1);
+    if (r0 == 0 && c4 < C4) {
+#pragma unroll
+      for (int j = 0; j < V; ++j) pout[2 * g.C + c4 * V + j] = u0[j];
+    }
+    return;
   }
   if (t.kind == NORM_TAIL_NONE) return;
 
@@ -611,7 +706,7 @@
                                                              NormGeom g, int ns, const NormTail t) {
   __shared__ double red[NORM_FB_NB][8][NORM_FB_CH];
   __shared__ double tn[NORM_FB_NB][NORM_FB_CH];
-  __shared__ double tot[3][NORM_FB_CH];
+  __shared__ double tot[5][NORM_FB_CH];
   const int tid = threadIdx.x;
   const int cl = tid & 3, kg = (tid >> 2) & 7, nl = tid >> 5, nlanes = (int)blockDim.x >> 5;
   const int c = blockIdx.x * NORM_FB_CH + cl;
@@ -624,8 +719,9 @@
       for (int nn = nl; nn < nb; nn += nlanes) {
         double acc = 0.0;
         if (cok) {
-          const double* src = part + (((size_t)(n0 + nn) * g.chunks) * 3 + sidx) * g.C + c;
-          const size_t kstride = (size_t)3 * g.C;
+          const double* src = sidx < 3 ? part + (((size_t)(n0 + nn) * g.chunks) * 3 + sidx) * g.C + c
+                                       : t.xpart + (((size_t)(n0 + nn) * g.chunks) * 2 + (sidx - 3)) * g.C + c;
+          const size_t kstride = (size_t)(sidx < 3 ? 3 : 2) * g.C;
 #pragma unroll 4
           for (int k = kg; k < g.chunks; k += 8) acc += src[k * kstride];
         }
@@ -639,7 +735,7 @@
 #pragma unroll
           for (int j = 0; j < 8; ++j) s8 += red[nn][j][cl];
           tn[nn][cl] = s8;
-          if (cok) nc[((size_t)sidx * g.N + n0 + nn) * g.C + c] = s8;
+          if (cok && sidx < 3) nc[((size_t)sidx * g.N + n0 + nn) * g.C + c] = s8;
         }
       }
       __syncthreads();
@@ -677,6 +773,8 @@
     t.k3[c] = (float)(-r * m1 + r * r * m2 * mu);
     if (t.dgamma) t.dgamma[c] = (float)sx;
     if (t.dbeta) t.dbeta[c] = (float)a0;
+    if (t.dbias)
+      t.dbias[c] = (float)((double)t.k1[c] * tot[3][tid] + (double)t.k2[c] * tot[4][tid] + (double)t.k3[c] * tot[2][tid]);
   } else {
     t.colsum[c] = (float)a0;
   }
@@ -910,6 +1008,38 @@
   return MSEG_OK;
 }
 
+extern "C" int mseg_norm_bwd_coeffs_supported(int st_, int act, int norm) {
+  return st_ == MSEG_ST_F32 && norm == MSEG_NORM_BN && (act == MSEG_ACT_NONE || act == MSEG_ACT_RELU);
+}
+
+extern "C" int mseg_norm_bwd_coeffs(const void* gy, const void* z, int N, int HW, int C, int st_, int act, int norm,
+                                    const float* gamma, const float* mean, const float* rstd, float* k1, float* k2,
+                                    float* k3, float* dgamma, float* dbeta, float* dbias, void* ws, void* stream) {
+  if (!gy || !z || !mean || !rstd || !k1 || !k2 || !k3 || !ws || N <= 0 || HW <= 0 || C <= 0 || (C & 3)) return MSEG_EINVAL;
+  if (!mseg_norm_bwd_coeffs_supported(st_, act, norm)) return MSEG_EINVAL;
+  hipStream_t st = (hipStream_t)stream;
+  NormGeom g = norm_geom(N, HW, C, 4);
+  NormGeom g4 = g, g8 = norm_geom(N, HW, C, 8);
+  const int chunks_max = g4.chunks > g8.chunks ? g4.chunks : g8.chunks;
+  double* part = (double*)((char*)ws + NORM_CTR_BYTES);
+  double* nc = part + (size_t)N * g.chunks * 3 * C;
+  NormTail t = {};
+  t.kind = NORM_TAIL_NONE;
+  t.norm = norm; t.ctr = (unsigned*)ws; t.nc = nc; t.gamma = gamma; t.mean = mean; t.rstd = rstd;
+  t.k1 = k1; t.k2 = k2; t.k3 = k3; t.dgamma = dgamma; t.dbeta = dbeta; t.dbias = dbias;
+  t.xpart = part + (size_t)N * chunks_max * 3 * C + (size_t)3 * N * C + (size_t)2 * N * C + (size_t)32 * C;
+  hipLaunchKernelGGL((norm_pass_kernel<1, false, false, true>), dim3(g.chunks, N, g.slices), dim3(256), 0, st, z, gy,
+                     (void*)nullptr, (const float*)nullptr, (const float*)nullptr, (const float*)nullptr, 0, g, act, part,
+                     (void*)nullptr, t);
+  MSEG_LAUNCH_CHECK();
+  NormTail tf = t;
+  tf.kind = NORM_TAIL_BN_BWD;
+  hipLaunchKernelGGL(norm_bn_finish_kernel, dim3((unsigned)((C + NORM_FB_CH - 1) / NORM_FB_CH)), dim3(N > 8 ? 1024 : 256), 0,
+                     st, (const double*)part, nc, g, dbias ? 5 : 2, tf);
+  MSEG_LAUNCH_CHECK();
+  return MSEG_OK;
+}
+
 __global__ void maxpool_fwd_kernel(const MsegSrc s, int N, int H, int W, float* __restrict__ out) {
   const int Ho = H >> 1, Wo = W >> 1, C4 = s.C >> 2;
   const size_t total = (size_t)N * Ho * Wo * C4;
diff --git a/microbeseg_amd/engine.py b/microbeseg_amd/engine.py
--- a/microbeseg_amd/engine.py
+++ b/microbeseg_amd/engine.py
@@ -352,13 +352,14 @@
 
 
 class KernelChoice:
-    __slots__ = ("name", "bf16", "launches", "grid", "block", "workspace", "stats_rows")
+    __slots__ = ("name", "bf16", "launches", "grid", "block", "workspace", "stats_rows", "dz_on_load")
 
     def __init__(self, info):
         self.name = info.name.decode()
         self.bf16 = info.precision == 1
         self.launches, self.grid, self.block, self.workspace = info.launches, info.grid, info.block, info.workspace
         self.stats_rows = info.stats_rows
+        self.dz_on_load = bool(info.dz_on_load)
 
     def __repr__(self):
         return f"KernelChoice({self.name!r}, bf16={self.bf16}, grid={self.grid})"
@@ -384,8 +385,24 @@
     return KernelChoice(info) if rc == 0 else None
 
 
+class DzOnLoad:
+    __slots__ = ("z", "k", "kss", "act", "out")
+
+    def __init__(self, z, k, kss, act, out):
+        self.z, self.k, self.kss, self.act, self.out = z, k, kss, act, out
+
+    def fill(self, p):
+        if self.k is None:
+            p.dz_z = p.dz_k1 = p.dz_k2 = p.dz_k3 = p.dz_out = _DUMMY
+        else:
+            step = self.k.numel() // 3 * 4
+            p.dz_z, p.dz_out = self.z.data_ptr(), self.out.data_ptr()
+            p.dz_k1, p.dz_k2, p.dz_k3 = self.k.data_ptr(), self.k.data_ptr() + step, self.k.data_ptr() + 2 * step
+        p.dz_kss, p.dz_act = self.kss, self.act
+
+
 def igemm_query(srcs, kpad, npad, NB, Hi, Wi, Ho, Wo, KH, KW, stride, pad, mode, Ngemm, ld0, acc0=0, ld1=0, acc1=0,
-                split=None, epi=EPI_PLAIN, Cq=0, morder=MORDER_LINEAR, precision=None, dst_dtype=ST_F32, bias=True):
+                split=None, epi=EPI_PLAIN, Cq=0, morder=MORDER_LINEAR, precision=None, dst_dtype=ST_F32, bias=True, dz=None):
     p = MsegIgemm()
     _fill_igemm(p, srcs, kpad, npad, NB, Hi, Wi, Ho, Wo, KH, KW, stride, pad, mode, Ngemm, ld0, acc0, ld1, acc1, split, epi, Cq,
                 morder)
@@ -394,6 +411,8 @@
     p.bias = _DUMMY if bias else None
     p.precision = 1 if (precision or _precision) == "bf16" else 0
     p.dst_dtype = dst_dtype
+    if dz is not None:
+        dz.fill(p)
     return _query(_lib.load().mseg_igemm_query, p)
 
 
@@ -422,7 +441,7 @@
 
 def igemm(srcs, w, bias, NB, Hi, Wi, Ho, Wo, KH, KW, stride, pad, mode, Ngemm, dst0, ld0, acc0=0,
           dst1=None, ld1=0, acc1=0, split=None, epi=EPI_PLAIN, Cq=0, morder=MORDER_LINEAR, real_cin=None,
-          precision=None, stats=None):
+          precision=None, stats=None, dz=None):
     lib = _lib.load()
     p = MsegIgemm()
     _fill_igemm(p, srcs, w.Kpad, w.Npad, NB, Hi, Wi, Ho, Wo, KH, KW, stride, pad, mode, Ngemm, ld0, acc0, ld1, acc1, split, epi,
@@ -436,6 +455,8 @@
     if bf16:
         p.w = w.bf16().data_ptr()
     p.precision = 1 if bf16 else 0
+    if dz is not None:
+        dz.fill(p)
     need = lib.mseg_igemm_workspace_bytes(C.byref(p))
     if need:
         key = (dst0.device, _stream())
@@ -599,6 +620,22 @@
                             node.mean.data_ptr(), node.rstd.data_ptr(), gy.data_ptr(), _ptr(dgamma), _ptr(dbeta),
                             _ptr(dbias), _ptr(node.a), w.data_ptr(), _stream()), "norm_bwd")
     return gy
+
+
+def norm_bwd_coeffs_ok(node):
+    return node.a is None and bool(_lib.load().mseg_norm_bwd_coeffs_supported(_st(node.z), node.act, node.norm))
+
+
+def norm_bwd_coeffs(node, gy, gamma, dgamma, dbeta, dbias, ws):
+    lib = _lib.load()
+    N, HW, Cc = node.N, node.H * node.W, node.C
+    w = ws.get("norm", lib.mseg_norm_workspace_bytes(N, HW, Cc), zero=True)
+    k = ws.get("norm_k", 3 * Cc * 4)[:3 * Cc * 4].view(torch.float32).view(3, 1, Cc)
+    kp = k.data_ptr()
+    check(lib.mseg_norm_bwd_coeffs(gy.data_ptr(), node.z.data_ptr(), N, HW, Cc, _st(node.z), node.act, node.norm, _ptr(gamma),
+                                   node.mean.data_ptr(), node.rstd.data_ptr(), kp, kp + 4 * Cc, kp + 8 * Cc, _ptr(dgamma),
+                                   _ptr(dbeta), _ptr(dbias), w.data_ptr(), _stream()), "norm_bwd_coeffs")
+    return k
 
 
 class ConvSpec:
@@ -898,6 +935,35 @@
     return _wgrad_overlap
 
 
+_dz_on_load = os.environ.get("MSEG_DZ_ON_LOAD", "1") != "0"
+_dz_ok_cache = {}
+
+
+def set_dz_on_load(flag):
+    global _dz_on_load
+    _dz_on_load = bool(flag)
+
+
+def get_dz_on_load():
+    return _dz_on_load
+
+
+def _dz_on_load_ok(node, cout, cin, ins):
+    if not _dz_on_load or _precision != "fp32" or node.z.dtype != torch.float32 or not norm_bwd_coeffs_ok(node):
+        return False
+    i0 = ins[0]
+    key = (node.N, node.H, node.W, cout, cin, tuple(i.C for i in ins), node.act)
+    ok = _dz_ok_cache.get(key)
+    if ok is None:
+        npad, kpad = _dummy_pack(cin, cout)
+        kw = {} if len(ins) == 1 else dict(ld1=ins[1].C, split=i0.C)
+        choice = igemm_query([_dummy_src(cout, ST_F32)], kpad, npad, node.N, node.H, node.W, i0.H, i0.W, 3, 3, 1, 1, MODE_TCONV,
+                             cin, i0.C if len(ins) > 1 else cin, precision="fp32", bias=False,
+                             dz=DzOnLoad(None, None, 0, node.act, None), **kw)
+        ok = _dz_ok_cache[key] = choice is not None and choice.dz_on_load
+    return ok
+
+
 _overlap_in_capture = os.environ.get("MSEG_OVERLAP_IN_CAPTURE", "0") == "1"
 
 
@@ -1000,7 +1066,15 @@
         dgamma = _grad_buf(nm.weight, direct) if has_affine else None
         dbeta = _grad_buf(nm.bias, direct) if has_affine else None
         dbias = _grad_buf(conv.bias, direct)
-        dz = norm_bwd(node, gy, nm.weight.detach() if has_affine else None, dgamma, dbeta, dbias, ws)
+        gamma = nm.weight.detach() if has_affine else None
+        dzl = None
+        if sp.kind == "conv" and node.inputs[0] is not tape.x4 and \
+                _dz_on_load_ok(node, conv.weight.shape[0], conv.weight.shape[1], node.inputs):
+            k = norm_bwd_coeffs(node, gy, gamma, dgamma, dbeta, dbias, ws)
+            dz = torch.empty_like(gy)
+            dzl = DzOnLoad(node.z, k, 0, node.act, dz)
+        else:
+            dz = norm_bwd(node, gy, gamma, dgamma, dbeta, dbias, ws)
         if has_affine:
             grads[id(nm.weight)] = dgamma
             grads[id(nm.bias)] = dbeta
@@ -1022,28 +1096,34 @@
             cout, cin = wt.shape[0], wt.shape[1]
             stride = 2 if sp.kind == "pool" else 1
             is_first = i0 is tape.x4
-            if is_first and cin == 1 and _first_layer_ok(cin, cout, stride):
-                w1 = ws.get("first_wgrad", lib.mseg_first_wgrad_workspace_bytes(N, node.H, node.W, cout))
-                check(lib.mseg_first_wgrad(i0.z.data_ptr(), dz.data_ptr(), _st(dz), N, node.H, node.W, cout, dW.data_ptr(),
-                                           w1.data_ptr(), _stream()), "first_wgrad")
-            else:
-                on_side(dz, lambda w_, dz=dz, ins=ins, dW=dW, cout=cout, node=node, i0=i0, stride=stride, cin=cin,
-                        is_first=is_first: wgrad(plain_src(dz, cout), [n.src() for n in ins], dW, N, node.H, node.W, i0.H,
-                                                 i0.W, 3, 3, stride, 1, w_, nch_store=cin if is_first else None))
+            def run_wgrad():
+                if is_first and cin == 1 and _first_layer_ok(cin, cout, stride):
+                    w1 = ws.get("first_wgrad", lib.mseg_first_wgrad_workspace_bytes(N, node.H, node.W, cout))
+                    check(lib.mseg_first_wgrad(i0.z.data_ptr(), dz.data_ptr(), _st(dz), N, node.H, node.W, cout,
+                                               dW.data_ptr(), w1.data_ptr(), _stream()), "first_wgrad")
+                else:
+                    on_side(dz, lambda w_, dz=dz, ins=ins, dW=dW, cout=cout, node=node, i0=i0, stride=stride, cin=cin,
+                            is_first=is_first: wgrad(plain_src(dz, cout), [n.src() for n in ins], dW, N, node.H, node.W,
+                                                     i0.H, i0.W, 3, 3, stride, 1, w_, nch_store=cin if is_first else None))
+            if dzl is None:
+                run_wgrad()
             if not is_first:
                 wp = pack_weight(conv.weight, 9, cin, cout, 1, 9, cin * 9, kind="dgrad")
                 morder = MORDER_PARITY if stride == 2 else MORDER_LINEAR
+                src = plain_src(gy if dzl is not None else dz, cout)
                 if len(ins) == 1:
                     tgt, acc = _accumulate_target(i0, None)
-                    igemm([plain_src(dz, cout)], wp, None, N, node.H, node.W, i0.H, i0.W, 3, 3, stride, 1,
-                          MODE_TCONV, cin, tgt, cin, acc0=acc, morder=morder)
+                    igemm([src], wp, None, N, node.H, node.W, i0.H, i0.W, 3, 3, stride, 1,
+                          MODE_TCONV, cin, tgt, cin, acc0=acc, morder=morder, dz=dzl)
                 else:
                     i1 = ins[1]
                     t0, a0 = _accumulate_target(i0, None)
                     t1, a1 = _accumulate_target(i1, None)
-                    igemm([plain_src(dz, cout)], wp, None, N, node.H, node.W, i0.H, i0.W, 3, 3, stride, 1,
+                    igemm([src], wp, None, N, node.H, node.W, i0.H, i0.W, 3, 3, stride, 1,
                           MODE_TCONV, cin, t0, i0.C, acc0=a0, dst1=t1, ld1=i1.C, acc1=a1,
-                          split=i0.C, morder=morder)
+                          split=i0.C, morder=morder, dz=dzl)
+            if dzl is not None:
+                run_wgrad()
         grads[id(conv.weight)] = dW
         if on_grads is not None:
             on_grads([dW, dbias, dgamma, dbeta])
```
